# slimgroup/SetIntersectionProjection.jl

Measured on AMD Instinct MI355X. Metric: PARSDMM iterations/sec, higher is better.
Workload: dtype f32

## Files before the change

include/sipx.h:

```cpp
#ifndef SIPX_H
#define SIPX_H

#include <stdint.h>

#ifdef __cplusplus
extern "C" {
#endif

typedef struct sipx_ctx sipx_ctx;

enum { SIPX_F32 = 0, SIPX_F64 = 1 };

enum { SIPX_OP_IDENTITY = 0, SIPX_OP_DX = 1, SIPX_OP_DY = 2, SIPX_OP_DZ = 3, SIPX_OP_TV = 4,
       SIPX_OP_CSC = 5 ,
       SIPX_OP_TV_XY = 6  };

enum {
  SIPX_PROJ_BOUNDS      = 0,
  SIPX_PROJ_BOUNDS_VEC  = 1,
  SIPX_PROJ_L1          = 2,
  SIPX_PROJ_L2          = 3,
  SIPX_PROJ_ANNULUS     = 4,
  SIPX_PROJ_CARDINALITY = 5,
  SIPX_PROJ_PROX_L1     = 6,
// ... 60 lines not shown

const char* sipx_last_error(void);

int sipx_create(sipx_ctx** out, int dtype, int ndim, const int64_t* n, const double* h, int device);
void sipx_destroy(sipx_ctx* ctx);

int sipx_add_set(sipx_ctx* ctx, const sipx_set_desc* desc, const void* ata_R, const int64_t* ata_off, int d_i);

int sipx_set_rows(sipx_ctx* ctx, int set, int64_t* rows);
int sipx_num_terms(sipx_ctx* ctx, int* p, int* pp);

int sipx_finalize(sipx_ctx* ctx, const void* m, const double* rho_ini, int n_rho, double gamma_ini,
                  int feasibility_only, int zero_ini_guess, const void* x0, const void* const* l0,
                  const void* const* y0, double* feasibility_initial);

int sipx_reset(sipx_ctx* ctx, const void* m, const double* rho_ini, int n_rho, double gamma_ini, int zero_ini_guess,
               const void* x0, const void* const* l0, const void* const* y0, double* feasibility_initial);

int sipx_rhs_compose(sipx_ctx* ctx, const double* rho);
int sipx_argmin_x(sipx_ctx* ctx, int it, double* tol_ref_io, int64_t* cg_it, double* cg_relres, int* cg_flag);
enum { SIPX_YL_FEAS = 1,
       SIPX_YL_BB = 2,
       SIPX_YL_FIRST = 4   };
int sipx_update_y_l(sipx_ctx* ctx, int it, int flags, const double* rho, const double* gamma,
                    double* r_pri, double* r_dual, double* feas );
int sipx_log_scalars(sipx_ctx* ctx, double* obj, double* evol_x);
int sipx_adapt_rho_gamma(sipx_ctx* ctx, int adjust_rho, int adjust_gamma, double* rho_io, double* gamma_io);
int sipx_q_update(sipx_ctx* ctx, const double* rho_new, const double* rho_old);
int sipx_download(sipx_ctx* ctx, void* x, void* const* l, void* const* y);

int sipx_set_caller_stream(sipx_ctx* ctx, void* stream);
int sipx_finalize_dev(sipx_ctx* ctx, const void* m, const double* rho_ini, int n_rho, double gamma_ini, int feasibility_only,
                      int zero_ini_guess, const void* x0, const void* const* l0, const void* const* y0,
                      double* feasibility_initial);
int sipx_reset_dev(sipx_ctx* ctx, const void* m, const double* rho_ini, int n_rho, double gamma_ini, int zero_ini_guess,
                   const void* x0, const void* const* l0, const void* const* y0, double* feasibility_initial);
int sipx_download_dev(sipx_ctx* ctx, void* x, void* const* l, void* const* y);

int sipx_set_data(sipx_ctx* ctx, int set, const void* lb, const void* ub);
int sipx_set_data_dev(sipx_ctx* ctx, int set, const void* lb, const void* ub);
int sipx_io_bytes(sipx_ctx* ctx, int64_t* host_to_device, int64_t* device_to_host, int reset);

int sipx_warm_start_from(sipx_ctx* fine, sipx_ctx* coarse);

int sipx_parsdmm(sipx_ctx* ctx, const sipx_options* opt, sipx_log* log);
int sipx_parsdmm_begin(sipx_ctx* ctx, const sipx_options* opt, sipx_log* log);
int sipx_parsdmm_steps(sipx_ctx* ctx, int nsteps, int* done);

int sipx_cds_spmv(int dtype, int64_t N, int d, const void* R, const int64_t* off, const void* x, void* y, int device);
int sipx_apply_op(sipx_ctx* ctx, int op, const void* x, void* s);
int sipx_apply_op_adj(sipx_ctx* ctx, int op, const void* v, void* t);
int sipx_project(sipx_ctx* ctx, const sipx_set_desc* desc, void* v, int64_t len);
int sipx_segment_norms(sipx_ctx* ctx, int op, int mode, int dir, int norm, const void* x, void* out, int64_t* nseg);
int sipx_segment_norms_dev(sipx_ctx* ctx, int op, int mode, int dir, int norm, const void* x, void* out, int64_t* nseg);
int sipx_l21_norm(sipx_ctx* ctx, const void* x, void* out);
int sipx_l21_norm_dev(sipx_ctx* ctx, const void* x, void* out);
int sipx_l21_norms(sipx_ctx* ctx, int op, int mode, int dir, const void* x, void* out, int64_t* nseg);
int sipx_l21_norms_dev(sipx_ctx* ctx, int op, int mode, int dir, const void* x, void* out, int64_t* nseg);
int sipx_l21_joint_norm(sipx_ctx* ctx, const void* x, void* out);
int sipx_l21_joint_norm_dev(sipx_ctx* ctx, const void* x, void* out);
int sipx_l21_weighted_norm(sipx_ctx* ctx, int op, int joint, const void* x, const void* w, void* out);
int sipx_l21_weighted_norm_dev(sipx_ctx* ctx, int op, int joint, const void* x, const void* w, void* out);
int sipx_resample_nn(int dtype, int ndim, const int64_t* nc, const int64_t* nf, const void* in, void* out, int device);
int sipx_dwt(int dtype, int ndim, const int64_t* n, int inverse, const void* in, void* out, int device);

typedef struct {
  void* nuclear_norm; void* nuclear_Dx; void* nuclear_Dz; void* rank_095; void* TV; void* wavelet_l1; void* Dx_l1;
  void* Dz_l1; void* DFT_l1; void* DFT_card_095; void* TV_card_095; void* annulus; void* TV_annulus; void* D_l2;
  void* D_x_min; void* D_x_max; void* D_z_min; void* D_z_max; void* DCT_x_LB; void* DCT_x_UB; void* DCT_y_LB;
  void* DCT_y_UB; void* hist_min; void* hist_max; void* hist_TV_min; void* hist_TV_max;
} sipx_observations;
int sipx_learn_observations(int dtype, const int64_t* n, const double* h, int64_t n_train, const void* m_train,
                            const int64_t* strides, int64_t max_batch, sipx_observations* out, int device);
int sipx_get_Q(sipx_ctx* ctx, void* Q, int64_t* offsets, int* d);
int sipx_q_terms(sipx_ctx* ctx, int* bands, int* matrix_free);
int sipx_time_spmv(sipx_ctx* ctx, int reps, double* avg_ms);
int sipx_kernel_stats(sipx_ctx* ctx, int enable, int64_t* launches, double* total_ms);
const char* sipx_kernel_stats_json(sipx_ctx* ctx, int enable);
int sipx_debug_proj(sipx_ctx* ctx, int set, int which, double* out16);
void* sipx_stream(sipx_ctx* ctx);
void* sipx_dev_rhs(sipx_ctx* ctx);
void* sipx_dev_x(sipx_ctx* ctx);
int sipx_get_rhs(sipx_ctx* ctx, void* rhs);
int sipx_prox_l2s(int dtype, int64_t n, void* x, double rho, const void* m, int device);
int sipx_set_owned(sipx_ctx* ctx, const int32_t* owned);

int sipx_rccl_unique_id(void* id128);
#define SIPX_DECOMP_SETS 0
#define SIPX_DECOMP_SLAB 1
#define SIPX_DECOMP_SLAB_FULL 2
int sipx_set_decomp(sipx_ctx* ctx, int mode);
int sipx_set_comm_rccl(sipx_ctx* ctx, const void* id128, int world, int rank);
typedef struct {
  void* user;
  int32_t world, rank;
  int (*allreduce_sum)(void* user, void* buf, int64_t count, int32_t dtype, void* stream);
  int (*reduce_scatter_sum)(void* user, void* buf, int64_t chunk, int32_t dtype, void* stream);
  int (*allgather)(void* user, void* buf, int64_t chunk, int32_t dtype, void* stream);
  int (*halo_exchange)(void* user, const void* send_prev, void* recv_prev, int32_t prev, const void* send_next, void* recv_next,
                       int32_t next, int64_t count, int32_t dtype, void* stream);
  int (*scatter)(void* user, void* buf, int64_t chunk, int32_t dtype, int32_t root, void* stream);
  int (*gather)(void* user, void* buf, int64_t chunk, int32_t dtype, int32_t root, void* stream);
} sipx_comm;
int sipx_set_comm(sipx_ctx* ctx, const sipx_comm* comm);
int sipx_comm_info(sipx_ctx* ctx, int* nranks, int* rank, char* version, int version_len, int* decomposition);
int sipx_device_bytes(sipx_ctx* ctx, int64_t* context_bytes, int64_t* device_used, int64_t* device_total);
int sipx_slab(sipx_ctx* ctx, int64_t* row0, int64_t* row1, int64_t* chunk);

enum { SIPX_Q_CDS = 0, SIPX_Q_STENCIL = 1 };
int sipx_set_q_mode(sipx_ctx* ctx, int mode);
int sipx_apply_Q(sipx_ctx* ctx, const void* x, void* y);

#ifdef __cplusplus
}
#endif
#endif
```

setintersectionprojection.jl_amd/csrc/api.cpp:

```cpp
#include <string>

#include "comm.h"
#include "engine.h"
#include "learn.h"

struct sipx_ctx {
  sipx::EngineBase* e;
};

static thread_local std::string g_err;

#define SIPX_TRY(body)                   \
  try {                                  \
    body;                                \
    return 0;                            \
  } catch (const std::exception& ex) {   \
    g_err = ex.what();                   \
    return 1;                            \
  } catch (...) {                        \
    g_err = "unknown error";             \
    return 1;                            \
  }

extern "C" {
// ... 75 lines not shown
  SIPX_TRY({
    if (!fine || !coarse) throw std::runtime_error("null context");
    fine->e->warm_start_from(coarse->e);
  })
}
int sipx_parsdmm(sipx_ctx* c, const sipx_options* opt, sipx_log* log) { SIPX_TRY(c->e->parsdmm(opt, log)) }
int sipx_parsdmm_begin(sipx_ctx* c, const sipx_options* opt, sipx_log* log) { SIPX_TRY(c->e->parsdmm_begin(opt, log)) }
int sipx_parsdmm_steps(sipx_ctx* c, int nsteps, int* done) {
  SIPX_TRY({
    bool d = false;
    for (int k = 0; k < nsteps && !d; ++k) d = c->e->parsdmm_step();
    if (done) *done = d ? 1 : 0;
  })
}

int sipx_cds_spmv(int dtype, int64_t N, int d, const void* R, const int64_t* off, const void* x, void* y, int device) {
  SIPX_TRY(sipx::refresh_env_knobs(); sipx::cds_spmv_host(dtype, N, d, R, off, x, y, device))
}
int sipx_resample_nn(int dtype, int ndim, const int64_t* nc, const int64_t* nf, const void* in, void* out, int device) {
  SIPX_TRY(sipx::refresh_env_knobs(); sipx::resample_nn_host(dtype, ndim, nc, nf, in, out, device))
}
int sipx_dwt(int dtype, int ndim, const int64_t* n, int inverse, const void* in, void* out, int device) {
  SIPX_TRY(sipx::refresh_env_knobs(); sipx::dwt_host(dtype, ndim, n, inverse, in, out, device))
}
int sipx_learn_observations(int dtype, const int64_t* n, const double* h, int64_t n_train, const void* m_train,
                            const int64_t* strides, int64_t max_batch, sipx_observations* out, int device) {
  SIPX_TRY(sipx::refresh_env_knobs(); sipx::learn_observations_host(dtype, n, h, n_train, m_train, strides, max_batch, out, device))
}
int sipx_apply_op(sipx_ctx* c, int op, const void* x, void* s) { SIPX_TRY(c->e->apply_op(op, x, s, false)) }
int sipx_apply_op_adj(sipx_ctx* c, int op, const void* v, void* t) { SIPX_TRY(c->e->apply_op(op, v, t, true)) }
int sipx_project(sipx_ctx* c, const sipx_set_desc* d, void* v, int64_t len) { SIPX_TRY(sipx::refresh_env_knobs(); c->e->project(d, v, len)) }
int sipx_segment_norms(sipx_ctx* c, int op, int mode, int dir, int norm, const void* x, void* out, int64_t* nseg) {
  SIPX_TRY(sipx::refresh_env_knobs(); c->e->segment_norms(op, mode, dir, norm, x, out, nseg, false))
}
int sipx_segment_norms_dev(sipx_ctx* c, int op, int mode, int dir, int norm, const void* x, void* out, int64_t* nseg) {
  SIPX_TRY(sipx::refresh_env_knobs(); c->e->segment_norms(op, mode, dir, norm, x, out, nseg, true))
}
int sipx_l21_norm(sipx_ctx* c, const void* x, void* out) {
  SIPX_TRY(sipx::refresh_env_knobs(); c->e->l21_norms(SIPX_PROJ_L21, SIPX_OP_TV, SIPX_MODE_WHOLE, 0, x, out, nullptr, false, false))
}
int sipx_l21_norm_dev(sipx_ctx* c, const void* x, void* out) {
  SIPX_TRY(sipx::refresh_env_knobs(); c->e->l21_norms(SIPX_PROJ_L21, SIPX_OP_TV, SIPX_MODE_WHOLE, 0, x, out, nullptr, true, false))
}
int sipx_l21_norms(sipx_ctx* c, int op, int mode, int dir, const void* x, void* out, int64_t* nseg) {
  SIPX_TRY(sipx::refresh_env_knobs(); c->e->l21_norms(SIPX_PROJ_L21, op, mode, dir, x, out, nseg, false, true))
}
int sipx_l21_norms_dev(sipx_ctx* c, int op, int mode, int dir, const void* x, void* out, int64_t* nseg) {
  SIPX_TRY(sipx::refresh_env_knobs(); c->e->l21_norms(SIPX_PROJ_L21, op, mode, dir, x, out, nseg, true, true))
}
int sipx_l21_joint_norm(sipx_ctx* c, const void* x, void* out) {
  SIPX_TRY(sipx::refresh_env_knobs(); c->e->l21_norms(SIPX_PROJ_L21_JOINT, SIPX_OP_TV_XY, SIPX_MODE_WHOLE, 0, x, out, nullptr, false, false))
}
int sipx_l21_joint_norm_dev(sipx_ctx* c, const void* x, void* out) {
  SIPX_TRY(sipx::refresh_env_knobs(); c->e->l21_norms(SIPX_PROJ_L21_JOINT, SIPX_OP_TV_XY, SIPX_MODE_WHOLE, 0, x, out, nullptr, true, false))
}
int sipx_l21_weighted_norm(sipx_ctx* c, int op, int joint, const void* x, const void* w, void* out) {
  SIPX_TRY(sipx::refresh_env_knobs(); c->e->l21_weighted_norm(op, joint != 0, x, w, out, false))
}
int sipx_l21_weighted_norm_dev(sipx_ctx* c, int op, int joint, const void* x, const void* w, void* out) {
  SIPX_TRY(sipx::refresh_env_knobs(); c->e->l21_weighted_norm(op, joint != 0, x, w, out, true))
}
int sipx_get_Q(sipx_ctx* c, void* Q, int64_t* offsets, int* d) { SIPX_TRY(c->e->get_Q(Q, offsets, d)) }
int sipx_q_terms(sipx_ctx* c, int* bands, int* matrix_free) { SIPX_TRY(c->e->q_terms(bands, matrix_free)) }
int sipx_time_spmv(sipx_ctx* c, int reps, double* avg_ms) { SIPX_TRY(*avg_ms = c->e->time_spmv(reps)) }
int sipx_kernel_stats(sipx_ctx* c, int enable, int64_t* launches, double* total_ms) {
  SIPX_TRY(c->e->kernel_stats(enable, launches, total_ms))
}
const char* sipx_kernel_stats_json(sipx_ctx* c, int enable) {
  try {
    return c->e->kernel_stats_json(enable);
  } catch (const std::exception& ex) {
    g_err = ex.what();
    return nullptr;
  } catch (...) {
    g_err = "unknown error";
    return nullptr;
  }
}
int sipx_debug_proj(sipx_ctx* c, int set, int which, double* out16) { SIPX_TRY(c->e->debug_proj(set, which, out16)) }
void* sipx_stream(sipx_ctx* c) { return c->e->stream(); }
void* sipx_dev_rhs(sipx_ctx* c) { return c->e->dev_rhs(); }
void* sipx_dev_x(sipx_ctx* c) { return c->e->dev_x(); }
int sipx_get_rhs(sipx_ctx* c, void* rhs) { SIPX_TRY(c->e->get_rhs(rhs)) }
int sipx_prox_l2s(int dtype, int64_t n, void* x, double rho, const void* m, int device) {
  SIPX_TRY(sipx::refresh_env_knobs(); sipx::prox_l2s_host(dtype, n, x, rho, m, device))
}
int sipx_set_owned(sipx_ctx* c, const int32_t* owned) { SIPX_TRY(c->e->set_owned(owned)) }
int sipx_rccl_unique_id(void* id128) { SIPX_TRY(sipx::rccl_unique_id(id128)) }
int sipx_set_comm_rccl(sipx_ctx* c, const void* id128, int world, int rank) {
  SIPX_TRY({
    sipx::refresh_env_knobs();
    c->e->bind_device();
    c->e->set_comm(sipx::make_rccl_comm(id128, world, rank));
  })
}
int sipx_set_comm(sipx_ctx* c, const sipx_comm* comm) {
  SIPX_TRY({
    if (!comm) throw std::runtime_error("null communicator");
    sipx::refresh_env_knobs();
    c->e->set_comm(sipx::make_callback_comm(comm));
  })
}
int sipx_comm_info(sipx_ctx* c, int* nranks, int* rank, char* version, int version_len, int* decomposition) {
  SIPX_TRY(c->e->comm_info(nranks, rank, version, version_len, decomposition))
}
int sipx_device_bytes(sipx_ctx* c, int64_t* context_bytes, int64_t* device_used, int64_t* device_total) {
  SIPX_TRY(c->e->device_bytes(context_bytes, device_used, device_total))
}
int sipx_slab(sipx_ctx* c, int64_t* row0, int64_t* row1, int64_t* chunk) { SIPX_TRY(c->e->slab(row0, row1, chunk)) }
int sipx_set_q_mode(sipx_ctx* c, int mode) { SIPX_TRY(c->e->set_q_mode(mode)) }
int sipx_set_decomp(sipx_ctx* c, int mode) { SIPX_TRY(c->e->set_decomp(mode)) }
int sipx_apply_Q(sipx_ctx* c, const void* x, void* y) { SIPX_TRY(c->e->apply_Q(x, y)) }

}
```

setintersectionprojection.jl_amd/csrc/engine.cpp:

```cpp
#include "engine.h"
#include "comm.h"
#include "device_memory.h"
#include "dist_dft.h"
#include "ext_proj.h"
#include "host_prefault.h"
#include "set_config.h"
#include "solve_rules.h"
#include "sparse_granules.h"

#include <algorithm>
#include <array>
#include <chrono>
#include <cmath>
#include <cstdio>
#include <cstdlib>
#include <cstring>
#include <limits>
#include <thread>
#include <exception>

namespace sipx {

const LaunchObserver*& launch_observer() {
  static thread_local const LaunchObserver* obs = nullptr;
// ... 745 lines not shown
        s.cbuf = mem_.alloc<T>(s.Mpad, Mem::State);
      }
    }
    if (s.prox == SIPX_PROJ_BOUNDS_VEC) {
      s.lb = mem_.alloc<T>(s.Mpad); s.ub = mem_.alloc<T>(s.Mpad);
      if (!s.pend_lb) upload_rows(s, s.host_lb.data(), s.lb);
      if (!s.pend_ub) upload_rows(s, s.host_ub.data(), s.ub);
      if (s.pend_lb || s.pend_ub) {
        IoArgs<T> A;
        if (s.pend_lb) io_add_bounds(A, s, s.pend_lb, s.lb);
        if (s.pend_ub) io_add_bounds(A, s, s.pend_ub, s.ub);
        io_rows<T>(stream_, A, false, NB);
      }
    }
    if (!dev_io_ && l0 && l0[i]) upload_rows_ranged(s, (const T*)l0[i], s.l);
    if (!dev_io_ && y0 && y0[i]) upload_rows_ranged(s, (const T*)y0[i], s.y);
  }

  void create_lane(const FinalizePlan& P) {
    const bool one_rank = !comm_ && !mk_ && sweep_partial_;
    const bool slabbed = comm_ && slab_ && slab_loose_ && !mk_ && sweep_partial_;
    lane_set_ = -1;
    if (env_knobs().rank_lane && (one_rank || slabbed))
      for (int i = 0; i < p_n_ && lane_set_ < 0; ++i) {
        const SetState<T>& s = sets_[i];
        if (s.owned && !s.in_sweep && (one_rank ? !s.dist_ext : s.slab_ext) && s.ident && !s.custom && s.ext && s.rank_like()) lane_set_ = i;
      }
    if (lane_set_ < 0) return;
    int pr_least = 0, pr_greatest = 0;
    SIPX_HIP(hipDeviceGetStreamPriorityRange(&pr_least, &pr_greatest));
    SIPX_HIP(hipStreamCreateWithPriority(&lane_st_, hipStreamNonBlocking, pr_greatest));
    SIPX_HIP(hipEventCreateWithFlags(&lane_fork_, hipEventDisableTiming));
    SIPX_HIP(hipEventCreateWithFlags(&lane_ev_, hipEventDisableTiming));
    if (slab_) lane_v_ = (slab_local_ && !loose_whole_) ? loose_alloc(P.Npad) : mem_.alloc<T>((size_t)std::max<long long>(P.fullpad, sets_[lane_set_].Mpad), Mem::State);
    else lane_v_ = mem_.alloc<T>((size_t)sets_[lane_set_].Mpad, Mem::State);
  }

  void reset(const void* m, const double* rho_ini, int n_rho, double gamma_ini, int zero_ini_guess, const void* x0,
             const void* const* l0, const void* const* y0, double* feasibility_initial) override {
    need_final();
    if (comm_) throw std::runtime_error("sipx_reset is not available for a rank of a sharded solve (build a new context)");
    SIPX_HIP(hipSetDevice(device_));
    if (lane_thr_.joinable()) lane_thr_.join();
    lane_err_ = nullptr;
    SIPX_HIP(hipStreamSynchronize(stream_));
    for (hipStream_t q : pool_) if (q && q != stream_) SIPX_HIP(hipStreamSynchronize(q));
    if (lane_st_) SIPX_HIP(hipStreamSynchronize(lane_st_));
    if (cstream_) SIPX_HIP(hipStreamSynchronize(cstream_));
    const long long N = G_.N;
    mem_.zero_state(stream_);
    if (!dev_io_) {
      SIPX_HIP(hipMemcpyAsync(m_, m, N * sizeof(T), hipMemcpyHostToDevice, stream_));
      io_h2d_ += N * (long long)sizeof(T);
    }
    x_cur_ = 0; x_snap_ = -1;
    x_ = xr_[0]; xold_ = x_;
    init_rho_gamma(rho_ini, n_rho, gamma_ini);
    const bool warm = !zero_ini_guess;
    for (int i = 0; i < p_n_; ++i) {
      SetState<T>& s = sets_[i];
      s.snap = -1;
      s.searches_done = 0;
      std::fill(s.sums, s.sums + SLOTS, 0.0);
      s.bb_valid = false;
      s.last_rho = T(-1); s.last_gamma = T(-1);
      if (s.ps) K<T>::ps_init(stream_, s.ps, scr_i_);
      if (s.psf) K<T>::ps_init(stream_, s.psf, scr_i_);
      if (s.ext) { s.ext->set_stream(stream_); s.ext->reset(); }
      if (warm && !dev_io_ && l0 && l0[i]) upload_rows_ranged(s, (const T*)l0[i], s.l);
      if (warm && !dev_io_ && y0 && y0[i]) upload_rows_ranged(s, (const T*)y0[i], s.y);
    }
    if (dev_io_) {
      import_dev(m, warm ? x0 : nullptr, warm ? l0 : nullptr, warm ? y0 : nullptr);
    } else if (warm && x0) {
      SIPX_HIP(hipMemcpyAsync(x_, x0, Nx_ * sizeof(T), hipMemcpyHostToDevice, stream_));
      io_h2d_ += Nx_ * (long long)sizeof(T);
    }
    for (const PinnedBlock& b : pinned_blocks()) std::memset(*b.p, b.fill, b.bytes);
    sums_seq_ = 0; cg_seq_ = 0; spec_seq_ = 0;
    spec_searches_ = spec_fallbacks_ = spec_rounds_ = 0;
    batch_searches_ = batch_fallbacks_ = 0;
    for (long long& c : routes_) c = 0;
    head_done_ = false; rs_pending_ = false; sums_pending_ = false; merged_nslots_ = 0;
    rhs_fused_ = false; have_log_sums_ = false;
    obj_ss_ = evo_ss_ = xx_ss_ = 0;
    sums_flags_ = 0;
    marks_.reset();
    run_ = Run();
    assemble_Q();
    build_q_table();
    initial_feasibility(feasibility_initial);
  }

  void initial_feasibility(double* feasibility_initial) {
    feas_init_.assign(pp_n_, 0.0);
    for (int i = 0; i < pp_n_; ++i) {
      SetState<T>& s = sets_[i];
      if (s.dist_ext || s.slab_ext || s.slab_dft) {
        dist_feasibility(s, m_, fe2_part(i), i);
        continue;
      }
      if (s.fan) {
        SetArgs<T> a = set_args(s, rho_[i], gamma_[i], 0);
        a.x = m_;
        fan_feasibility(s, a, fe2_part(i));
        continue;
      }
      if (!s.owned) continue;
      if (slab_local_ && !s.two_pass && !s.ext_kind && !s.custom) {
        SetArgs<T> a = set_args(s, rho_[i], gamma_[i], 0);
        a.x = m_;
        K<T>::proj_dist_set(stream_, Gr_, a, 1, (const ProjScalars<T>*)nullptr, fe2_part(i));
        continue;
      }
      if (slab_ && !s.two_pass && comm_->rank != 0) continue;
      double* dst = fe2_part(i);
      const T* mm = s.comp == 2 ? w_ : m_;
      if (s.ext_kind) {
        SetArgs<T> a = set_args(s, rho_[i], gamma_[i], 0);
        a.x = mm;
        ext_feasibility(s, a, dst);
      } else if (s.custom) {
        custom_fwd(stream_, s, mm, s.sbuf);
        if (s.two_pass) {
          SetArgs<T> a = set_args(s, rho_[i], gamma_[i], 0);
          a.x = s.sbuf;
          K<T>::proj_scalars_set(stream_, s.gm, a, 1, s.psf, part_tmp_, maxpart_, scr_c_, s.Mtrue);
          K<T>::proj_dist_set(stream_, s.gm, a, 1, s.psf, dst);
        } else {
          proj_dist_grid<T>(stream_, s.gm, 0, s.dir, s.Mpad, s.sbuf, s.prox, s.plo, s.phi, s.lb, s.ub, nullptr, dst);
        }
      } else if (s.two_pass) {
        SetArgs<T> a = set_args(s, rho_[i], gamma_[i], 0);
        a.x = mm;
        SampleCtl cf;
        cf.host_ovf = (int*)hovf_ + i;
        cf.compact_cap = scr_c_len_;
        K<T>::proj_scalars_set(stream_, Gr_, a, 1, s.psf, part_tmp_, maxpart_, scr_c_, s.Mtrue, cf, hooks());
        K<T>::proj_dist_set(stream_, Gr_, a, 1, s.psf, dst);
      } else {
        K<T>::fwd(stream_, G_, s.nblk, s.dir, s.ih, mm, scr_v_);
        proj_dist_grid<T>(stream_, G_, s.nblk, s.dir, s.Mpad, scr_v_, s.prox, s.plo, s.phi, s.lb, s.ub, nullptr, dst);
      }
    }
    reduce_set_sums(p_n_ * SLOTS, YlPlan::Route::ByEvent);
    SIPX_HIP(hipStreamSynchronize(stream_));
    for (int i = 0; i < p_n_ && slab_; ++i)
      if (hovf_[i]) {
        hovf_[i] = 0;
        throw std::runtime_error("initial feasibility of set " + std::to_string(i) + ": the magnitudes inside the final bracket of the " + std::string(sets_[i].prox == PX_CARD ? "cardinality" : "l1") +
                                 " search, gathered over all ranks, exceed the exchange segment of " +
                                 std::to_string(hooks_.gcap) + " values per rank (slab decomposition) -- use the set decomposition for this problem");
      }
    for (int i = 0; i < pp_n_; ++i) {
      if (!sets_[i].owned && !comm_) continue;
      feas_init_[i] = (double)feas_value(hres_[i * SLOTS + SL_FE2], hres_[i * SLOTS + SL_SS2]);
    }
    if (feasibility_initial)
      for (int i = 0; i < pp_n_; ++i) feasibility_initial[i] = feas_init_[i];
  }

  void rhs_compose(const double* rho) override {
    need_final();
    ObserverGuard og(observer());
    head_done_ = false;
    if (rs_pending_) {
      SIPX_HIP(hipStreamWaitEvent(stream_, ev_c_[1], 0));
      rs_pending_ = false;
    }
    if (mk_) {
      for (int half = 0; half < 2; ++half) {
        T* out = rhs_ + (long long)half * G_.N;
        RhsBatch b(stream_, G_, out, false);
        for (int pass = 0; pass < 2; ++pass) {
          for (int i = 0; i < p_n_; ++i)
            if (sets_[i].comp == (pass == 0 ? half + 1 : 3)) b.add(sets_[i], (T)rho[i]);
          b.finish();
        }
        if (b.launched == 0) SIPX_HIP(hipMemsetAsync(out, 0, G_.N * sizeof(T), stream_));
      }
      return;
    }
    RhsBatch b(stream_, Gr_, rhs_, false);
    for (int i = 0; i < p_n_; ++i)
      if (sets_[i].owned && !sets_[i].custom) b.add(sets_[i], (T)rho[i]);
    if (b.launched == 0) b.flush();
    else b.finish();
    for (int i = 0; i < p_n_; ++i) {
      const SetState<T>& s = sets_[i];
      if (s.owned && s.custom) custom_adj_rhs(stream_, s, (T)rho[i]);
    }
    if (comm_ && !slab_) {
      SIPX_HIP(hipEventRecord(ev_c_[0], stream_));
      SIPX_HIP(hipStreamWaitEvent(cstream_, ev_c_[0], 0));
      comm_->reduce_scatter_sum(rhs_, (size_t)chunk_, dtype_code(), cstream_);
      SIPX_HIP(hipEventRecord(ev_c_[1], cstream_));
      rs_pending_ = true;
    }
  }

  void argmin_x_head() {
    if (rs_pending_) {
      SIPX_HIP(hipStreamWaitEvent(stream_, ev_c_[1], 0));
      rs_pending_ = false;
    }
    const long long r0 = r0_, r1 = r1_;
    const int dt = dtype_code();
    if (stencil_q_) K<T>::sq_resid(stream_, G_, sq_, x_, rhs_, p_, (T*)nullptr, (T*)nullptr, part_cg_);
    else K<T>::resid(stream_, Nx_, r0, r1, Q_, cds_, x_, rhs_, p_, (T*)nullptr, (T*)nullptr, part_cg_);
    mf_terms(x_, p_,  T(-1),  2, nullptr, nullptr);
    if (comm_) {
      comm_->allreduce_with_halo(part_cg_, (size_t)(2 * NB + merged_nslots_), SIPX_F64, p_ + r0, p_ + r0 - plane_, prev_, p_ + r1 - plane_,
                                 p_ + r1, next_, (size_t)plane_, dt, stream_);
      if (merged_nslots_ > 0) K<T>::copy_f64(stream_, dres_, hres_, merged_nslots_);
      merged_nslots_ = 0;
    }
    head_done_ = true;
  }

  void argmin_x(int it, double* tol_ref_io, int64_t* cg_it, double* cg_relres, int* cg_flag) override {
    need_final();
    ObserverGuard og(observer());
    if (!head_done_) argmin_x_head();
    head_done_ = false;
    const long long r0 = r0_, r1 = r1_, nloc = r1 - r0;
    const int dt = dtype_code();
    const long long hlo = (comm_ && prev_ >= 0) ? plane_ : 0, hhi = (comm_ && next_ >= 0) ? plane_ : 0;
    const unsigned seq = ++cg_seq_;
    K<T>::cg_begin(stream_, part_cg_, cg_dev_, cg_host_, it, (T)*tol_ref_io, seq, (unsigned long long*)ticket_);
    int tgt = 0;
    while (tgt == x_cur_ || tgt == x_snap_) ++tgt;
    T* const xn = xr_[tgt];
    auto enqueue = [&](int k) {
      CgState<T>* mirror = cg_host_ + (k & 1);
      if (stencil_q_) K<T>::sq_spmv_dot(stream_, G_, sq_, p_, Ap_, part_cg_, cg_dev_);
      else K<T>::spmv_dot(stream_, Nx_, r0, r1, Q_, cds_, p_, Ap_, part_cg_, cg_dev_);
      mf_terms(p_, Ap_, T(1),  1, p_, &cg_dev_->done);
      if (comm_) comm_->allreduce_sum(part_cg_, NB, SIPX_F64, stream_);
      K<T>::cg_update_xr(stream_, nloc, (k == 1 ? x_ : xn) + r0, xn + r0, (k == 1 ? p_ : r_) + r0, r_ + r0, p_ + r0, Ap_ + r0, part_cg_, cg_dev_, mirror, k,
                         (unsigned long long*)ticket_, hlo, hhi);
      if (comm_)
        comm_->allreduce_with_halo(part_cg_ + NB, NB, SIPX_F64, r_ + r0, r_ + r0 - plane_, prev_, r_ + r1 - plane_, r_ + r1, next_,
                                   (size_t)plane_, dt, stream_);
      K<T>::cg_update_p(stream_, nloc, p_ + r0, r_ + r0, part_cg_, cg_dev_, mirror, (unsigned long long*)ticket_, hlo, hhi);
    };
    auto enqueue_fused = [&](int k) {
      CgState<T>* mirror = cg_host_ + (k & 1);
      T* pk = (k & 1) ? p_ : p2_;
      T* pn = (k & 1) ? p2_ : p_;
      if (k == 1) K<T>::spmv_dot(stream_, Nx_, r0, r1, Q_, cds_, p_, Ap_, part_cg_, cg_dev_);
      K<T>::cg_update_xr(stream_, nloc, k == 1 ? x_ : xn, xn, k == 1 ? p_ : r_, r_, pk, Ap_, part_cg_, cg_dev_, mirror, k, (unsigned long long*)ticket_);
      K<T>::spmv_fused(stream_, Nx_, Q_, cds_, r_, pk, pn, Ap_, part_cg_, cg_dev_, mirror, (unsigned long long*)ticket_);
    };
    const size_t stat0 = samples_.size();
    const bool ahead = it > 1;
    auto enq = [&](int k) { if (cg_fused_) enqueue_fused(k); else enqueue(k); };
    if (ahead) enq(1);
    bool done = wait_ticket(seq, 0, cg_host_);
    const bool done_at_begin = done;
    CgState<T> fin;
    if (done) {
      fin = cg_host_[0];
      drop_samples_from(stat0);
      if (fin.flag == -9) SIPX_HIP(hipMemsetAsync(xn + r0 - hlo, 0, (nloc + hlo + hhi) * sizeof(T), stream_));
    } else {
      const int maxIter = 1000;
      int iter = 1;
      if (!ahead) enq(1);
      for (;;) {
        done = wait_ticket(seq, iter, cg_host_ + (iter & 1));
        if (done || iter == maxIter) break;
        enq(++iter);
      }
      fin = cg_host_[iter & 1];
    }
    cg_host_[0] = fin;
    const bool wrote = fin.flag == -9 || (!done_at_begin && !(fin.flag == -2 && fin.iters <= 1));
    if (wrote) {
      xold_ = x_;
      x_cur_ = tgt;
      x_ = xn;
    } else {
      xold_ = x_;
    }
// ... 964 lines not shown
        if (!s.two_pass || !s.in_sweep || s.prox != PX_L1 || s.custom || s.ext_kind) continue;
        SetArgs<T> a = set_args(s, (T)rho[i], (T)gamma[i], flags);
        if (a.flags & F_NOSPEC) continue;
        const bool rescaled = s.rescaled(a.rho);
        if (rescaled || search_ctl(i, rescaled, true).enable) { ok = false; break; }
        if (lm.ns == LEAN_MAX) break;
        const SetScratch scr = scratch_of(s);
        LeanSet<T>& S = lm.s[lm.ns++];
        S.a = a; S.a.ps = s.ps; S.ps = s.ps;
        S.compact = scr.cbuf; S.partials = scr.ptmp; S.maxpart = scr.mpart;
        who.push_back(i);
      }
      bool own = true;
      for (int i : who) own &= sets_[i].ptmp != nullptr && sets_[i].mpart != nullptr && sets_[i].cbuf != nullptr;
      if (ok && own && lm.ns >= 2) {
        K<T>::lean_multi(stream_, Gr_, lm);
        for (int i : who) lean_done[i] = 1;
      }
    }
    if (set_streams_) SIPX_HIP(hipEventRecord(ev_fork_, stream_));
    for (int i = 0; i < p_n_; ++i) {
      SetState<T>& s = sets_[i];
      if (!s.two_pass || !s.in_sweep) continue;
      SetArgs<T> a = set_args(s, (T)rho[i], (T)gamma[i], flags);
      hipStream_t q = s.st ? s.st : stream_;
      const SetScratch scr = scratch_of(s);
      if (q != stream_) SIPX_HIP(hipStreamWaitEvent(q, ev_fork_, 0));
      const bool rescaled = s.rescaled(a.rho);
      if (rescaled) K<T>::ps_rescale(q, s.ps, s.rescale_factor(a.rho));
      SampleCtl ctl = search_ctl(i, rescaled, true);
      ctl.lean_done = lean_done[i];
      K<T>::proj_scalars_set(q, Gr_, a, 0, s.ps, scr.ptmp, scr.mpart, scr.cbuf, s.Mtrue, ctl, nullptr);
      s.last_rho = a.rho;
      s.last_gamma = a.gamma;
      if (feas && i < pp_n_) {
        SampleCtl cf;
        cf.runs = env_knobs().l1_sample_runs;
        cf.enable = env_knobs().l1_sample && a.prox == PX_L1;
        K<T>::proj_scalars_set(q, Gr_, a, 1, s.psf, scr.ptmp, scr.mpart, scr.cbuf, s.Mtrue, cf, nullptr);
        K<T>::proj_dist_set(q, Gr_, a, 1, s.psf, fe2_part(i));
      }
    }
    join_set_streams([this](int i) { return sets_[i].two_pass && sets_[i].in_sweep; });
  }

  void sweep_launch(int flags, const double* rho, const double* gamma, MultiArgs<T>& ma, bool fuse_rhs) {
    const bool first = (flags & SIPX_YL_FIRST) != 0, bb = (flags & SIPX_YL_BB) != 0 && !first;
    ma.nblk = 0;
    std::vector<int> target(p_n_, 0);
    bool behind = false;
    for (int i = 0; i < p_n_; ++i) {
      SetState<T>& s = sets_[i];
      if (!s.in_sweep) { behind = true; target[i] = -1; continue; }
      SetArgs<T> a = set_args(s, (T)rho[i], (T)gamma[i], flags);
      target[i] = (!first && !bb && s.snap == 1) ? 2 : 0;
      if (target[i] == 2 && !s.y2) throw std::runtime_error("internal: the third y / l pair of the sweep was not allocated at sipx_finalize");
      T* ty = target[i] == 2 ? s.y2 : s.y0;
      T* tl = target[i] == 2 ? s.l2 : s.l0;
      for (int qb = 0; qb < s.nblk_or1(); ++qb) {
        MultiBlk<T>& B = ma.b[ma.nblk++];
        const long long off = (long long)qb * G_.N;
        B.y = s.y + off; B.l = s.l + off;
        B.yo = ty + off; B.lo = tl + off;
        B.lh0 = s.lh0 + off; B.s0 = s.s0 + off;
        B.y0 = a.y0 + off; B.l0 = a.l0 + off;
        B.ps = s.ps;
        B.dir = s.nblk == 0 ? -1 : s.dir[qb];
        B.set = i;
        B.first = qb == 0;
        B.last = qb == s.nblk_or1() - 1;
        B.dist = s.is_dist ? 1 : 0;
        B.feas_el = (i < pp_n_ && (s.prox == PX_BOUNDS || s.prox == PX_PROX_L1)) ? 1 : 0;
        B.ih = s.nblk == 0 ? T(0) : s.ih[qb];
        B.rho = a.rho; B.rho1 = a.rho1; B.gamma = a.gamma;
        B.prox = s.prox; B.plo = s.plo; B.phi = s.phi;
        B.in_rhs = behind ? 0 : 1;
      }
    }
    ma.x = x_; ma.m = m_; ma.xold = xold_;
    ma.x0 = (x0_mode_ && x_snap_ >= 0) ? xr_[x_snap_] : (x0_mode_ ? x_ : nullptr);
    ma.x0w = nullptr;
    ma.rhs = fuse_rhs ? rhs_ : nullptr;
    ma.partials = part_sets_;
    if (!K<T>::yl_multi(stream_, G_, ma)) throw std::runtime_error("internal: the fused y/l sweep refused a block list it was prepared for");
    rhs_fused_ = ma.rhs != nullptr;
    if (x0_mode_ && (first || bb)) x_snap_ = x_cur_;
    for (int i = 0; i < p_n_; ++i) {
      SetState<T>& s = sets_[i];
      if (target[i] < 0) continue;
      if (target[i] == 2) {
        std::swap(s.y, s.y2); std::swap(s.l, s.l2);
      } else {
        std::swap(s.y, s.y0); std::swap(s.l, s.l0);
        if (first || bb) s.snap = 0;
        else if (s.snap == 0) s.snap = 1;
      }
    }
  }

  void collect_set_sums(YlPlan::Route route, const double* rho, double* r_pri, double* r_dual, double* feas) {
    if (!sums_pending_) throw std::runtime_error("no y/l update is pending");
    sums_pending_ = false;
    const int flags = sums_flags_;
    if (route == YlPlan::Route::ByWord) wait_word(sums_word_, sums_seq_);
    else SIPX_HIP(hipEventSynchronize(sums_event_));
    have_log_sums_ = false;
    if (slab_) {
      for (int i = 0; i < p_n_; ++i) {
        if (!hovf_[i]) continue;
        for (int k = 0; k <= p_n_; ++k) hovf_[k] = 0;
        ProjScalars<T> h;
        SIPX_HIP(hipStreamSynchronize(stream_));
        char dbg[512];
        int at = 0;
        for (const ProjScalars<T>* d : {sets_[i].ps, sets_[i].psf}) {
          if (!d) continue;
          SIPX_HIP(hipMemcpy(&h, d, sizeof(h), hipMemcpyDeviceToHost));
          if (!h.gather_overflow) continue;
          at += std::snprintf(dbg + at, sizeof dbg - at, " [%s: bracket (%.9g, %.9g], refinement rounds %d, ||v||_1 %.6g, radius %.6g, speculative range (%.9g, %.9g]]",
                              d == sets_[i].ps ? "y/l update" : "feasibility estimate", h.lo, h.hi, h.rounds_used, h.asum, (double)sets_[i].phi, h.spec_lo, h.spec_hi);
        }
        dbg[at] = 0;
        throw std::runtime_error(std::string(sets_[i].prox == PX_CARD ? "cardinality search" : "l1 threshold search") + " of set " + std::to_string(i) + ": the magnitudes inside the final bracket, gathered over all "
                                 "ranks, exceed the exchange segment of " + std::to_string(hooks_.gcap) + " values per rank "
                                 "(slab decomposition) after the refinement rounds of the search; the iterate of this step is not valid -- "
                                 "use the set decomposition for this problem" + std::string(dbg));
      }
    }
    const bool all = comm_ != nullptr;
    for (int i = 0; i < p_n_; ++i) {
      SetState<T>& s = sets_[i];
      if (r_pri) r_pri[i] = 0;
      if (r_dual) r_dual[i] = 0;
      if (!s.owned && !all) continue;
      const double* h = hres_ + (size_t)i * SLOTS;
      std::copy(h, h + SLOTS, s.sums);
      if (r_pri) r_pri[i] = (double)(T)std::sqrt(h[SL_RPRI]);
      if (r_dual) r_dual[i] = (double)((T)rho[i] * (T)std::sqrt((s.comp == 3 ? 2.0 : 1.0) * (s.ident ? h[SL_DY] : h[SL_ADJ])));
      s.bb_valid = (flags & (SIPX_YL_BB | SIPX_YL_FIRST)) != 0;
      if (s.is_dist) {
        obj_ss_ = h[SL_OBJ]; evo_ss_ = h[SL_EVO]; xx_ss_ = h[SL_XX];
        if (mk_) { evo_ss_ = hres_[(size_t)p_n_ * SLOTS + SL_EVO]; xx_ss_ = hres_[(size_t)p_n_ * SLOTS + SL_XX]; }
        have_log_sums_ = true;
      }
    }
    if (all && !slab_dist_logs_) {
      const double* g = hres_ + (size_t)p_n_ * SLOTS;
      obj_ss_ = g[SL_OBJ]; evo_ss_ = g[SL_EVO]; xx_ss_ = g[SL_XX];
      have_log_sums_ = true;
    }
    if ((flags & SIPX_YL_FEAS) && feas) {
      for (int i = 0; i < pp_n_; ++i) {
        feas[i] = 0;
        if (!sets_[i].owned && !all) continue;
        const double* h = hres_ + (size_t)i * SLOTS;
        feas[i] = (sets_[i].two_pass || sets_[i].ext_kind) ? (double)feas_value(h[SL_FE2], h[SL_SS2])
                                                            : (double)feas_value(h[SL_FE], h[SL_SS]);
      }
    }
  }

  void log_scalars(double* obj, double* evol_x) override {
    need_final();
    ObserverGuard og(observer());
    if (!have_log_sums_) {
      K<T>::log3(stream_, G_.N, mk_ ? w_ : x_, m_, xold_, part_sets_);
      if (mk_) K<T>::log3(stream_, Nx_, x_, (const T*)nullptr, xold_, part_sets_ + (size_t)SLOTS * NB);
      K<T>::fin_sum(stream_, part_sets_, (mk_ ? 2 : 1) * SLOTS, nullptr, hres_);
// ... 430 lines not shown
      const long long c0 = slab_local_ ? std::max<long long>(0, wlo_) : 0, c1 = slab_local_ ? std::min<long long>(G_.N, whi_) : G_.N;
      if (c1 > c0) SIPX_HIP(hipMemcpyAsync(x_ + c0, m_ + c0, (c1 - c0) * sizeof(T), hipMemcpyDeviceToDevice, stream_));
    }
    if (mk_) SIPX_HIP(hipMemsetAsync(x_ + G_.N, 0, G_.N * sizeof(T), stream_));
    SIPX_HIP(hipStreamSynchronize(stream_));
    log->n_iter = 1;
    log->n_feas_rows = 1;
    log->stopped_feasible = 1;
    run_.done = true;
  }

  bool parsdmm_step() override {
    Run& R = run_;
    if (!R.active) throw std::runtime_error("sipx_parsdmm_steps: call sipx_parsdmm_begin first");
    if (R.done) return true;
    ObserverGuard og(observer());
    const int i = ++R.i;
    begin_step(i);
    x_step(i);
    const YlPlan plan = yl_step(i);
    queue_ahead(i, plan);
    collect_set_sums(plan.route, R.rho.data(), R.rpri.data(), R.rdual.data(), R.feas.data());
    record_log_row(i);
    if (stop_rule(i)) {
      finish_solve(i);
      return true;
    }
    next_rho(i);
    apply_rho(i);
    if (i == R.maxit) finish_solve(i);
    return R.done;
  }

  void begin_step(int i) {
    marks_.resolve(run_.log, i & 1);
    marks_.begin_step(i);
  }

  void x_step(int i) {
    Run& R = run_;
    if (!head_done_) marks_.open(i);
    if (!R.rhs_ready) {
      rhs_compose(R.rho.data());
      marks_.mark(1);
    }
    R.rhs_ready = false;
    int64_t cg_it; double relres; int flag;
    argmin_x(i, &R.tol_ref, &cg_it, &relres, &flag);
    R.log->cg_it[i - 1] = cg_it;
    R.log->cg_relres[i - 1] = relres;
    marks_.mark(2);
  }

  YlPlan yl_step(int i) {
    Run& R = run_;
    YlPlan plan;
    plan.collect_now = false;
    plan.fuse_rhs = i < R.maxit && !rho_may_change<T>(R.sw, i, pp_n_, R.rho.data(), p_n_);
    if (comm_) plan.route = plan.fuse_rhs ? YlPlan::Route::WithNextHead : YlPlan::Route::ByEvent;
    else plan.route = marks_.stride > 1 ? YlPlan::Route::ByWord : YlPlan::Route::ByEvent;
    yl_update(i, yl_flags(R.sw, i), R.rho.data(), R.gamma.data(), plan);
    marks_.mark(3);
    if (plan.route != YlPlan::Route::ByWord) sums_event_here();
    return plan;
  }
  void sums_event_here() {
    sums_event_ = marks_.last_event();
    if (sums_event_) return;
    SIPX_HIP(hipEventRecord(ev_sums_, stream_));
    sums_event_ = ev_sums_;
  }

  void queue_ahead(int i, const YlPlan& plan) {
    Run& R = run_;
    if (rhs_fused_) {
      R.rhs_ready = true;
    } else if (plan.fuse_rhs) {
      rhs_compose(R.rho.data());
      marks_.mark(1);
      R.rhs_ready = true;
    }
    if (!R.rhs_ready) return;
    marks_.open(i + 1);
    argmin_x_head();
    if (comm_) {
      marks_.mark(-1);
      sums_event_here();
    }
  }

  void record_log_row(int i) {
    Run& R = run_;
    sipx_log* log = R.log;
    const int p = p_n_, pp = pp_n_;
    HostSection t(log->timing_ms[3]);
    for (int k = 0; k < p; ++k) {
      log->r_pri[(size_t)(i - 1) * p + k] = R.rpri[k];
      log->r_dual[(size_t)(i - 1) * p + k] = R.rdual[k];
      log->rho[(size_t)(i - 1) * p + k] = R.rho[k];
      log->gamma[(size_t)(i - 1) * p + k] = R.gamma[k];
    }
    log->r_dual_total[i - 1] = seq_sum<T>(R.rdual.data(), p);
    log->r_pri_total[i - 1] = seq_sum<T>(R.rpri.data(), p);
    if (feas_due(i)) {
      for (int k = 0; k < pp; ++k) log->set_feasibility[(size_t)(R.counter - 1) * pp + k] = R.feas[k];
      R.counter += 1;
    }
    log_scalars(&log->obj[i - 1], &log->evol_x[i - 1]);
  }

  bool stop_rule(int i) {
    Run& R = run_;
    HostSection t(R.log->timing_ms[4]);
    const LogView view{R.log->set_feasibility, R.log->obj, R.log->evol_x, R.log->r_pri_total};
    return sipx::stop_rule<T>(view, i, R.counter, pp_n_, R.tol, R.sw);
  }

  void next_rho(int i) {
    Run& R = run_;
    HostSection t(R.log->timing_ms[5]);
    R.rho_new = R.rho;
    if (bb_due(R.sw, i)) adapt_rho_gamma(R.sw.adjust_rho, R.sw.adjust_gamma, R.rho_new.data(), R.gamma.data());
    const double* latest = R.log->set_feasibility + (size_t)(R.counter - 2) * pp_n_;
    sipx::next_rho<T>(R.sw, i, pp_n_, latest, R.rho_new.data(), p_n_);
  }

  void apply_rho(int i) {
    Run& R = run_;
    if (R.rhs_ready && R.rho_new != R.rho) throw std::runtime_error("internal: rho changed under a right-hand side queued ahead");
    bool changed = false;
    for (int k = 0; k < p_n_; ++k) changed |= R.rho_new[k] != R.rho[k];
    const bool rhs_due = i < R.maxit && !R.rhs_ready;
    if (rhs_due || changed) marks_.mark(-1);
    if (rhs_due) {
      rhs_compose(R.rho_new.data());
      marks_.mark(1);
      R.rhs_ready = true;
    }
    if (changed) {
      q_update(R.rho_new.data(), R.rho.data());
      marks_.mark(6);
    }
    R.rho = R.rho_new;
  }

  void finish_solve(int n_iter) {
    Run& R = run_;
    if (rs_pending_) {
      SIPX_HIP(hipStreamWaitEvent(stream_, ev_c_[1], 0));
      rs_pending_ = false;
    }
    marks_.resolve(R.log, 0);
    marks_.resolve(R.log, 1);
    R.log->n_iter = n_iter;
    R.log->n_feas_rows = R.counter;
    for (int k = 0; k < p_n_; ++k) { rho_[k] = (T)R.rho[k]; gamma_[k] = (T)R.gamma[k]; }
    R.rhs_ready = false;
    R.done = true;
    head_done_ = false;
  }

  void parsdmm(const sipx_options* opt, sipx_log* log) override {
    parsdmm_begin(opt, log);
    while (!parsdmm_step()) {
    }
  }
// ... 305 lines not shown
                    "\"bytes_moved\": %.0f, \"gated\": %s, \"inclusive\": %s}",
                    first ? "" : ", ", kernel_name(k), (long long)agg[k].launches, (long long)agg[k].noops, agg[k].ms, agg[k].bytes_survey,
                    agg[k].bytes_moved,
                    gated ? "true" : "false", k == KID_EXT ? "true" : "false");
      o += buf;
      first = false;
    }
    o += "], \"slab_searches\": {\"speculative_exchange\": " + std::to_string(spec_searches_) + ", \"fallbacks\": " +
         std::to_string(spec_fallbacks_) + ", \"refinement_rounds\": " + std::to_string(spec_rounds_) + "}";
    o += std::string(", \"sparse_arrays\": ") + (slab_local_ ? "true" : "false");
    {
      std::string loc, fan;
      for (int i = 0; i < p_n_; ++i) {
        if (sets_[i].slab_ext || sets_[i].slab_card || sets_[i].slab_dft) loc += (loc.empty() ? "" : ", ") + std::to_string(i);
        if (sets_[i].fan) fan += (fan.empty() ? "" : ", ") + std::to_string(i);
      }
      if (counting_)
        o += ", \"collectives\": {\"allreduce\": " + std::to_string(counting_->n_allreduce) + ", \"allreduce_with_halo\": " + std::to_string(counting_->n_grouped) +
             ", \"allgather\": " + std::to_string(counting_->n_allgather) + ", \"reduce_scatter\": " + std::to_string(counting_->n_reduce_scatter) +
             ", \"halo\": " + std::to_string(counting_->n_halo) + ", \"scatter_gather\": " + std::to_string(counting_->n_fan) +
             ", \"alltoall\": " + std::to_string(counting_->n_alltoall) + "}";
      o += ", \"slab_loose\": {\"slab_local_sets\": [" + loc + "], \"gathered_sets\": [" + fan + "], \"fan_exchanges\": " + std::to_string(fan_exchanges_) + "}";
    }
    {
      std::string t = selftest_;
      for (auto& ch : t) if (ch == '"' || ch == '\\' || (unsigned char)ch < 32) ch = ' ';
      o += ", \"comm_selftest\": \"" + t + "\"";
    }
    o += ", \"lane_set\": " + std::to_string(lane_set_);
    o += std::string(", \"q_table\": {\"on\": ") + (cds_.qtab ? "true" : "false") + ", \"reason\": \"" + qtab_reason_ + "\"}";
    o += ", \"batched_searches\": {\"searches\": " + std::to_string(batch_searches_) + ", \"fallbacks\": " + std::to_string(batch_fallbacks_) + "}";
    o += ", \"routes\": {";
    for (int r = 0; r < RT_COUNT; ++r) o += std::string(r ? ", \"" : "\"") + route_name(r) + "\": " + std::to_string(routes_[r]);
    o += "}";
    long long rc[4] = {project_rc_[0], project_rc_[1], project_rc_[2], project_rc_[3]};
    for (const auto& st : sets_) {
      if (!st.ext || st.ext_kind != EXT_RANK) continue;
      long long c[4];
      st.ext->route_counts(c);
      for (int q = 0; q < 4; ++q) rc[q] += c[q];
    }
    o += ", \"rank_route\": {\"calls\": " + std::to_string(rc[0]) + ", \"warm_started_subspace\": " + std::to_string(rc[1]) +
         ", \"full_decomposition\": " + std::to_string(rc[2]) + ", \"products_with_gram\": " + std::to_string(rc[3]) + "}";
    long long fc[4] = {0, 0, 0, 0};
    for (const auto& st : sets_) {
      if (!st.ext || st.ext_kind != EXT_L21_SEG) continue;
      long long c[4];
      st.ext->route_counts(c);
      fc[0] += c[0]; fc[1] = std::max(fc[1], c[1]); fc[3] += c[3];
    }
    o += ", \"l21_frames\": {\"passes_total\": " + std::to_string(fc[0]) + ", \"passes_max\": " + std::to_string(fc[1]) +
         ", \"frames\": " + std::to_string(fc[3]) + "}";
    long long wc[4] = {0, 0, 0, 0};
    for (const auto& st : sets_) {
      if (!st.ext || !st.weighted) continue;
      long long c[4];
      st.ext->route_counts(c);
      for (int q = 0; q < 4; ++q) wc[q] += c[q];
    }
    o += ", \"l21_weighted\": {\"passes\": " + std::to_string(wc[0]) + ", \"flag_reads\": " + std::to_string(wc[1]) +
         ", \"calls\": " + std::to_string(wc[2]) + ", \"groups\": " + std::to_string(wc[3]) + "}}";
    if (!peek) start_stats(enable);
    return o.c_str();
  }
  double stat_pair_overhead_ms() const { return stat_pair_ms_; }

  void debug_proj(int set, int which, double* o) override {
    need_final();
    for (int k = 0; k < 16; ++k) o[k] = 0;
    if (set < 0 || set >= p_n_) throw std::runtime_error("set index out of range");
    const ProjScalars<T>* d = (which & 1) ? sets_[set].psf : sets_[set].ps;
    if (!d) return;
    ProjScalars<T> h;
    SIPX_HIP(hipStreamSynchronize(stream_));
    SIPX_HIP(hipMemcpy(&h, d, sizeof(h), hipMemcpyDeviceToHost));
    o[0] = h.need; o[1] = h.theta; o[2] = h.theta_prev; o[3] = h.hw; o[4] = h.spec_lo; o[5] = h.spec_hi; o[6] = h.lo;
    o[7] = h.hi; o[8] = h.asum; o[9] = h.vmax; o[10] = h.dbg[0]; o[11] = h.dbg[1]; o[12] = h.dbg[2]; o[13] = h.dbg[3];
    o[14] = h.refine;
    o[15] = h.lean + 2 * h.dbg_sampled;
    if (which & 2) { o[4] = h.samp_theta; o[5] = h.samp_lo; o[6] = h.samp_hi; o[7] = h.samp_c; }
  }

  void* stream() override { return (void*)stream_; }
  void* dev_rhs() override { return rhs_; }
  void* dev_x() override { return x_; }
  void get_rhs(void* out) override {
    need_final();
    if (slab_local_ && comm_->world > 1) throw std::runtime_error("a slab-decomposed context holds its planes of rhs only");
    SIPX_HIP(hipStreamSynchronize(stream_));
    SIPX_HIP(hipMemcpy(out, rhs_, Nx_ * sizeof(T), hipMemcpyDeviceToHost));
  }

 private:
  struct KSample { int kid; double bytes_survey, bytes_moved; };
  struct KAgg { long long launches = 0, noops = 0; double ms = 0, bytes_survey = 0, bytes_moved = 0; };
  hipEvent_t stat_event(size_t i) {
    while (stat_ev_.size() <= i) {
      hipEvent_t e;
      SIPX_HIP(hipEventCreate(&e));
      stat_ev_.push_back(e);
    }
    return stat_ev_[i];
  }
  static void obs_begin(void* user, int kid, hipStream_t s, double bytes_survey, double bytes_moved) {
    auto* e = static_cast<Engine<T>*>(user);
    if (e->stats_mode_ == 0 || (e->stats_mode_ == 1 && kid != KID_CDS_DOT && kid != KID_SQ_DOT)) return;
    const size_t i = e->samples_.size();
    e->samples_.push_back(KSample{kid, bytes_survey, bytes_moved});
    e->open_.push_back(i);
    SIPX_HIP(hipEventRecord(e->stat_event(2 * i), s));
  }
  static void obs_end(void* user, int kid, hipStream_t s) {
    auto* e = static_cast<Engine<T>*>(user);
    if (e->stats_mode_ == 0 || (e->stats_mode_ == 1 && kid != KID_CDS_DOT && kid != KID_SQ_DOT)) return;
    if (e->open_.empty()) return;
    const size_t i = e->open_.back();
    e->open_.pop_back();
    if (i < e->samples_.size()) SIPX_HIP(hipEventRecord(e->stat_event(2 * i + 1), s));
  }
  static void obs_route(void* user, int route) {
    if (route >= 0 && route < RT_COUNT) static_cast<Engine<T>*>(user)->routes_[route] += 1;
  }
  void drop_samples_from(size_t n) {
    if (n < samples_.size()) samples_.resize(n);
    open_.clear();
  }
  void sync_all_streams() {
    SIPX_HIP(hipStreamSynchronize(stream_));
    for (hipStream_t q : pool_) if (q != stream_) SIPX_HIP(hipStreamSynchronize(q));
    if (cstream_) SIPX_HIP(hipStreamSynchronize(cstream_));
  }
  static bool gated_kernel(int k) {
    return k == KID_PASS_FIRST || k == KID_PASS_LEAN || k == KID_PASS_PROBE || k == KID_PASS_COMPACT || k == KID_SAMPLE ||
           k == KID_DECIDE || k == KID_CDS_FUSED || k == KID_CG_XR || k == KID_CG_P || k == KID_SLOT_SUMS;
  }
  std::vector<KAgg> aggregate_samples() {
    sync_all_streams();
    std::vector<KAgg> agg(KID_COUNT);
    for (size_t i = 0; i < samples_.size(); ++i) {
      float ms = 0;
      if (hipEventElapsedTime(&ms, stat_ev_[2 * i], stat_ev_[2 * i + 1]) != hipSuccess) { (void)hipGetLastError(); continue; }
      KAgg& a = agg[samples_[i].kid];
      const double t = (double)ms - stat_pair_ms_;
      a.launches += 1;
      a.ms += t > 0 ? t : 0;
      const bool noop = gated_kernel(samples_[i].kid) && samples_[i].bytes_moved > 0 && t * 1e-3 < samples_[i].bytes_moved / 16e12;
      a.noops += noop ? 1 : 0;
      a.bytes_survey += noop ? 0.0 : samples_[i].bytes_survey;
      a.bytes_moved += noop ? 0.0 : samples_[i].bytes_moved;
    }
    return agg;
  }
  void start_stats(int mode) {
    samples_.clear();
    open_.clear();
    stats_mode_ = 0;
    if (mode) {
      std::vector<float> gap;
      for (int k = 0; k < 16; ++k) {
        SIPX_HIP(hipEventRecord(stat_event(2 * k), stream_));
        SIPX_HIP(hipEventRecord(stat_event(2 * k + 1), stream_));
      }
      SIPX_HIP(hipStreamSynchronize(stream_));
      for (int k = 0; k < 16; ++k) {
        float ms = 0;
        SIPX_HIP(hipEventElapsedTime(&ms, stat_ev_[2 * k], stat_ev_[2 * k + 1]));
        gap.push_back(ms);
      }
      std::sort(gap.begin(), gap.end());
      stat_pair_ms_ = gap[gap.size() / 2];
    }
    stats_mode_ = mode;
  }
// ... 502 lines not shown
    explicit DevIoGuard(bool* flag) : f(flag) { *f = true; }
    ~DevIoGuard() { *f = false; }
  };
  Grid G_;
  T ih_[3];
  std::vector<SetState<T>> sets_;
  std::vector<int32_t> owned_;
  bool finalized_ = false, feasibility_only_ = false, any_ncvx_ = false;
  int p_n_ = 0, pp_n_ = 0;
  std::vector<T> rho_, gamma_;
  std::vector<double> feas_init_;
  T *p_base_ = nullptr, *m_base_ = nullptr, *r_base_ = nullptr, *p2_base_ = nullptr, *p2_ = nullptr;
  bool cg_fused_ = false;
  int n_mfree_ = 0;
  long long halo_ = 0;
  T *x_ = nullptr, *xold_ = nullptr, *rhs_ = nullptr, *m_ = nullptr, *r_ = nullptr, *p_ = nullptr, *Ap_ = nullptr;
  T *Q_ = nullptr, *scr_v_ = nullptr, *scr_c_ = nullptr, *maxpart_ = nullptr;
  long long* scr_i_ = nullptr;
  long long scr_c_len_ = 0;
  T* scr_w_ = nullptr;
  T *loose_v_ = nullptr, *loose_w_ = nullptr;
  bool loose_whole_ = false;
  bool need_idx_ = false, need_ext_ = false;
  CdsArgs cds_;
  bool set_streams_ = true;
  hipEvent_t ev_fork_ = nullptr, ev_fork2_ = nullptr;
  std::vector<hipStream_t> pool_;
  bool search_streams_ = false;
  int search_next_ = 0;
  int n_set_streams_ = 2, pool_next_ = 0;
  bool mk_ = false;
  long long Nx_ = 0;
  T *w_base_ = nullptr, *w_ = nullptr;
  StencilQ<T> sq_{};
  bool stencil_q_ = false;
  double *part_cg_ = nullptr, *part_tmp_ = nullptr, *part_sets_ = nullptr;
  CgState<T>*cg_dev_ = nullptr, *cg_host_ = nullptr;
  double* hres_ = nullptr;
  volatile unsigned long long* sums_word_ = nullptr;
  unsigned* sums_ticket_ = nullptr;
  unsigned long long sums_seq_ = 0;
  volatile int* hlean_ = nullptr;
  volatile int* hovf_ = nullptr;
  volatile unsigned* hverd_ = nullptr;
  unsigned spec_seq_ = 0;
  long long spec_searches_ = 0, spec_fallbacks_ = 0, spec_rounds_ = 0;
  int lane_set_ = -1;
  hipStream_t lane_st_ = nullptr;
  hipEvent_t lane_fork_ = nullptr, lane_ev_ = nullptr;
  T* lane_v_ = nullptr;
  std::thread lane_thr_;
  std::exception_ptr lane_err_;
  long long lane_sample_ = -1;
  SetArgs<T> lane_args_;
  bool sweep_partial_ = false, has_loose_ = false;
  bool sweep_plain_ = false;
  bool search_batch_ = false;
  long long batch_searches_ = 0, batch_fallbacks_ = 0;
  long long routes_[RT_COUNT] = {};
  long long project_rc_[4] = {0, 0, 0, 0};
  T* fbuf_ = nullptr;
  bool yl_multi_ = true;
  bool x0_mode_ = false;
  T *xr_base_[3] = {nullptr, nullptr, nullptr}, *xr_[3] = {nullptr, nullptr, nullptr};
  int x_cur_ = 0, x_snap_ = -1;
  bool rhs_fused_ = false;
  hipEvent_t sums_event_ = nullptr;
  std::unique_ptr<Comm> comm_;
  CountingComm* counting_ = nullptr;
  long long plane_ = 0, chunk_ = 0, r0_ = 0, r1_ = 0, qr0_ = 0, qr1_ = 0;
  int prev_ = -1, next_ = -1;
  hipStream_t cstream_ = nullptr;
  hipEvent_t ev_c_[2] = {nullptr, nullptr};
  bool rs_pending_ = false;
  double* dres_ = nullptr;
  hipEvent_t ev_sums_ = nullptr, ev_cgb_ = nullptr;
  bool sums_pending_ = false;
  T* qtab_ = nullptr;
  bool q_stale_ = false;
  std::string qtab_reason_ = "not built";
  DeviceMemory mem_;
  bool slab_dist_logs_ = false;
  bool lean_multi_ = false;
  bool head_done_ = false;
  int merged_nslots_ = 0;
  int sums_flags_ = 0;
  volatile unsigned long long* ticket_ = nullptr;
  unsigned cg_seq_ = 0;
  bool slab_req_ = false, slab_ = false;
  hipStream_t fan_st_ = nullptr;
  hipEvent_t fan_fork_ = nullptr;
  double* fan_ptmp_ = nullptr;
  T *fan_mpart_ = nullptr, *fan_c_ = nullptr;
  long long fan_exchanges_ = 0;
  bool slab_loose_ = false;
  bool slab_full_req_ = false, slab_local_ = false;
  std::string selftest_ = "none", mapped_why_;
  double* agree_buf_ = nullptr;
  bool selftest_mapped_failed_ = false, selftest_alltoall_failed_ = false;
  std::string a2a_why_;
  long long wlo_ = 0, whi_ = 0;
  Grid Gr_, Gyl_;
  ChainHooks hooks_;
  T* gbuf_ = nullptr;
  double *stage_ = nullptr, *sstage_ = nullptr;
  const ChainHooks* hooks() const { return slab_ ? &hooks_ : nullptr; }
  double obj_ss_ = 0, evo_ss_ = 0, xx_ss_ = 0;
  bool have_log_sums_ = false;
  hipEvent_t cg_ev_[2] = {nullptr, nullptr};
  std::vector<hipEvent_t> stat_ev_;
  std::vector<KSample> samples_;
  std::vector<size_t> open_;
  int stats_mode_ = 0;
  LaunchObserver obs_{this, &Engine<T>::obs_begin, &Engine<T>::obs_end, &Engine<T>::obs_route};
  std::string stats_json_;
  double stat_pair_ms_ = 0;
};

EngineBase* make_engine(int dtype, int ndim, const int64_t* n, const double* h, int device) {
  const int count = hip_device_count();
  if (device < 0 || device >= count) throw std::runtime_error("libsipx: device index out of range");
  if (dtype == SIPX_F32) return new Engine<float>(ndim, n, h, device);
  if (dtype == SIPX_F64) return new Engine<double>(ndim, n, h, device);
  throw std::runtime_error("dtype must be SIPX_F32 or SIPX_F64");
}

template <typename T>
static void cds_spmv_T(int64_t N, int d, const void* R, const int64_t* off, const void* x, void* y) {
  if (d < 1 || d > MAXD) throw std::runtime_error("cds_spmv: band count out of range");
  long long H = 4;
  for (int b = 0; b < d; ++b) H = std::max<long long>(H, std::llabs((long long)off[b]));
  H = (H + 3) / 4 * 4;
  DeviceMemory tmp;
  T* dR = tmp.alloc<T>((size_t)N * d, Mem::NoFill);
  T* dxb = tmp.alloc<T>(N + 2 * H);
  T* dx = dxb + H;
  T* dy = tmp.alloc<T>(N);
  SIPX_HIP(hipMemcpy(dR, R, (size_t)N * d * sizeof(T), hipMemcpyHostToDevice));
  SIPX_HIP(hipMemcpy(dx, x, N * sizeof(T), hipMemcpyHostToDevice));
  CdsArgs a;
  a.d = d;
  for (int b = 0; b < d; ++b) a.off[b] = off[b];
  Grid g;
  g.n[0] = N; g.n[1] = 1; g.n[2] = 1; g.N = N; g.st[0] = 1; g.st[1] = N; g.st[2] = N;
  K<T>::spmv(nullptr, g, N, dR, a, dx, dy);
  SIPX_HIP(hipDeviceSynchronize());
  SIPX_HIP(hipMemcpy(y, dy, N * sizeof(T), hipMemcpyDeviceToHost));
}

template <typename T>
static void resample_T(int ndim, const int64_t* nc, const int64_t* nf, const void* in, void* out) {
  long long c[3] = {1, 1, 1}, f[3] = {1, 1, 1};
  for (int q = 0; q < ndim && q < 3; ++q) { c[q] = nc[q]; f[q] = nf[q]; }
  const long long Nc = c[0] * c[1] * c[2], Nf = f[0] * f[1] * f[2];
  if (Nc < 1 || Nf < 1) throw std::runtime_error("resample: empty array");
  DeviceMemory tmp;
  T* di = tmp.alloc<T>(Nc, Mem::NoFill);
  T* dout = tmp.alloc<T>(Nf, Mem::NoFill);
  SIPX_HIP(hipMemcpy(di, in, Nc * sizeof(T), hipMemcpyHostToDevice));
  resample_nn<T>(nullptr, c, f, di, dout);
  SIPX_HIP(hipDeviceSynchronize());
  SIPX_HIP(hipMemcpy(out, dout, Nf * sizeof(T), hipMemcpyDeviceToHost));
}
void resample_nn_host(int dtype, int ndim, const int64_t* nc, const int64_t* nf, const void* in, void* out, int device) {
  hip_device_count();
  if (ndim < 1 || ndim > 3) throw std::runtime_error("resample: ndim must be 1..3");
// ... 61 lines not shown
```

setintersectionprojection.jl_amd/csrc/engine.h:

```cpp
#pragma once
#include <memory>
#include <stdexcept>
#include <string>
#include <vector>

#include "../../include/sipx.h"
#include "sipx_common.h"

namespace sipx {

struct Comm;

struct EngineBase {
  virtual ~EngineBase() {}
  virtual int add_set(const sipx_set_desc* d, const void* ata_R, const int64_t* ata_off, int d_i) = 0;
  virtual int64_t set_rows(int set) = 0;
  virtual void num_terms(int* p, int* pp) = 0;
  virtual void finalize(const void* m, const double* rho_ini, int n_rho, double gamma_ini, int feasibility_only,
                        int zero_ini_guess, const void* x0, const void* const* l0, const void* const* y0,
                        double* feasibility_initial) = 0;
  virtual void reset(const void* m, const double* rho_ini, int n_rho, double gamma_ini, int zero_ini_guess, const void* x0,
                     const void* const* l0, const void* const* y0, double* feasibility_initial) = 0;
  virtual void rhs_compose(const double* rho) = 0;
  virtual void argmin_x(int it, double* tol_ref_io, int64_t* cg_it, double* cg_relres, int* cg_flag) = 0;
  virtual void update_y_l(int it, int flags, const double* rho, const double* gamma, double* r_pri, double* r_dual,
                          double* feas) = 0;
  virtual void log_scalars(double* obj, double* evol_x) = 0;
  virtual void adapt_rho_gamma(int adjust_rho, int adjust_gamma, double* rho_io, double* gamma_io) = 0;
  virtual void q_update(const double* rho_new, const double* rho_old) = 0;
  virtual void download(void* x, void* const* l, void* const* y) = 0;
  virtual void warm_start_from(EngineBase* coarse) = 0;
  virtual void finalize_dev(const void* m, const double* rho_ini, int n_rho, double gamma_ini, int feasibility_only,
                            int zero_ini_guess, const void* x0, const void* const* l0, const void* const* y0,
                            double* feasibility_initial) = 0;
  virtual void reset_dev(const void* m, const double* rho_ini, int n_rho, double gamma_ini, int zero_ini_guess, const void* x0,
                         const void* const* l0, const void* const* y0, double* feasibility_initial) = 0;
  virtual void download_dev(void* x, void* const* l, void* const* y) = 0;
  virtual void set_caller_stream(void* stream) = 0;
  virtual void set_data(int set, const void* lb, const void* ub, bool on_device) = 0;
  virtual void io_bytes(int64_t* host_to_device, int64_t* device_to_host, int reset) = 0;
  virtual void parsdmm(const sipx_options* opt, sipx_log* log) = 0;
  virtual void parsdmm_begin(const sipx_options* opt, sipx_log* log) = 0;
  virtual bool parsdmm_step() = 0;
  virtual void apply_op(int op, const void* x, void* s, bool adjoint) = 0;
  virtual void project(const sipx_set_desc* d, void* v, int64_t len) = 0;
  virtual void segment_norms(int op, int mode, int dir, int norm, const void* x, void* out, int64_t* nseg, bool on_device) = 0;
  virtual void l21_norms(int proj, int op, int mode, int dir, const void* x, void* out, int64_t* nseg, bool on_device, bool query) = 0;
  virtual void l21_weighted_norm(int op, bool joint, const void* x, const void* w, void* out, bool on_device) = 0;
  virtual void get_Q(void* Q, int64_t* offsets, int* d) = 0;
  virtual void apply_Q(const void* x, void* y) = 0;
  virtual void q_terms(int* bands, int* matrix_free) = 0;
  virtual double time_spmv(int reps) = 0;
  virtual void kernel_stats(int enable, int64_t* launches, double* total_ms) = 0;
  virtual const char* kernel_stats_json(int enable) = 0;
  virtual void debug_proj(int set, int which, double* out16) = 0;
  virtual void* stream() = 0;
  virtual void* dev_rhs() = 0;
  virtual void* dev_x() = 0;
  virtual void get_rhs(void* out) = 0;
  virtual void set_owned(const int32_t* owned) = 0;
  virtual void set_q_mode(int mode) = 0;
  virtual void set_decomp(int mode) = 0;
  virtual void set_comm(Comm* c) = 0;
  virtual void comm_info(int* nranks, int* rank, char* version, int version_len, int* decomposition) = 0;
  virtual void bind_device() = 0;
  virtual void device_bytes(int64_t* context_bytes, int64_t* device_used, int64_t* device_total) = 0;
  virtual void slab(int64_t* row0, int64_t* row1, int64_t* chunk) = 0;
};

EngineBase* make_engine(int dtype, int ndim, const int64_t* n, const double* h, int device);
void resample_nn_host(int dtype, int ndim, const int64_t* nc, const int64_t* nf, const void* in, void* out, int device);
void dwt_host(int dtype, int ndim, const int64_t* n, int inverse, const void* in, void* out, int device);
void prox_l2s_host(int dtype, int64_t n, void* x, double rho, const void* m, int device);
void cds_spmv_host(int dtype, int64_t N, int d, const void* R, const int64_t* off, const void* x, void* y, int device);

}
```

setintersectionprojection.jl_amd/csrc/kernels_cds.hip:

```cpp
#include <cstdlib>
#include <stdexcept>
#include <string>

#include "sipx_device.h"
#define SIPX_CG_GRID launch_blocks(3)
#ifndef SIPX_F64_VEC
#define SIPX_F64_VEC 2
#endif

namespace sipx {

template <typename T, int V>
struct LoadStored {
  const T* __restrict__ x;
  __device__ __forceinline__ Vec<T, V> operator()(long long c) const { return ldv_u<T, V>(x + c); }
};
template <typename T, int V>
struct LoadFused {
  const T* __restrict__ r;
  const T* __restrict__ p;
  T beta;
  __device__ __forceinline__ Vec<T, V> operator()(long long c) const {
    const Vec<T, V> rv = ldv_u<T, V>(r + c), pv = ldv_u<T, V>(p + c);
    Vec<T, V> o;
// ... 16 lines not shown
      if (a.sym) {
        rv[b] = a.off[b] >= 0 ? ldv<T, V>(R + (long long)b * N + r)
                              : ldv_u<T, V>(R + (long long)a.partner[b] * N + r + a.off[b]);
      } else {
        rv[b] = ldv_nt<T, V>(R + (long long)b * N + r);
      }
      xv[b] = xl(r + a.off[b]);
    }
#pragma unroll
    for (int b = 0; b < D; ++b) {
      const long long c = r + a.off[b];
#pragma unroll
      for (int k = 0; k < V; ++k) {
        const T t = acc[k] + rv[b].v[k] * xv[b].v[k];
        acc[k] = (c + k >= 0 && c + k < N) ? t : acc[k];
      }
    }
  } else {
    for (int b = 0; b < d; ++b) {
      const long long c = r + a.off[b];
      const Vec<T, V> rv = !a.sym ? ldv_nt<T, V>(R + (long long)b * N + r)
                                  : (a.off[b] >= 0 ? ldv<T, V>(R + (long long)b * N + r)
                                                   : ldv_u<T, V>(R + (long long)a.partner[b] * N + c));
      const Vec<T, V> xv = xl(c);
#pragma unroll
      for (int k = 0; k < V; ++k) {
        const T t = acc[k] + rv.v[k] * xv.v[k];
        acc[k] = (c + k >= 0 && c + k < N) ? t : acc[k];
      }
    }
  }
}

template <typename T, int V, int D, int MODE>
__global__ __launch_bounds__(BLOCK) void k_cds(long long N, long long r0, long long r1, const T* __restrict__ R, CdsArgs a,
                                               const T* __restrict__ x, T* __restrict__ y, const T* __restrict__ b,
                                               T* __restrict__ pout, T* __restrict__ xold, double* __restrict__ partials,
                                               const int* __restrict__ done) {
  if (MODE == 1 && *done) return;
  const long long nvec = r1 / V;
  double acc0 = 0, acc1 = 0;
  for (long long vi = r0 / V + (long long)blockIdx.x * BLOCK + threadIdx.x; vi < nvec; vi += (long long)gridDim.x * BLOCK) {
    const long long r = vi * V;
    T s[V];
    cds_rows<T, V, D>(N, R, a, LoadStored<T, V>{x}, r, s);
    if (MODE == 0) {
      Vec<T, V> o;
#pragma unroll
      for (int k = 0; k < V; ++k) o.v[k] = s[k];
      stv_nt<T, V>(y + r, o);
    } else if (MODE == 1) {
      const Vec<T, V> pv = ldv<T, V>(x + r);
      Vec<T, V> o;
#pragma unroll
      for (int k = 0; k < V; ++k) {
        o.v[k] = s[k];
        acc0 += (double)pv.v[k] * (double)s[k];
      }
      stv_nt<T, V>(y + r, o);
    } else {
      const Vec<T, V> bv = ldv<T, V>(b + r);
      const Vec<T, V> xv = ldv<T, V>(x + r);
      Vec<T, V> o;
#pragma unroll
      for (int k = 0; k < V; ++k) {
        o.v[k] = bv.v[k] - s[k];
        acc0 += (double)o.v[k] * (double)o.v[k];
        acc1 += (double)bv.v[k] * (double)bv.v[k];
      }
      stv<T, V>(y + r, o);
      if (pout) stv<T, V>(pout + r, o);
      if (xold) stv<T, V>(xold + r, xv);
    }
  }
  if (MODE == 1) {
    double acc[1] = {acc0};
    block_reduce_store<1>(acc, partials, 0);
  } else if (MODE == 2) {
    double acc[2] = {acc0, acc1};
    block_reduce_store<2>(acc, partials, 0);
  }
}

constexpr int march_role(int ord, int b) {
  constexpr int o1[7] = {0, 1, 2, 3, 4, 5, 6}, o2[7] = {0, 5, 3, 1, 2, 4, 6};
  return ord == 1 ? o1[b] : o2[b];
}
template <typename T>
__device__ __forceinline__ T ata_value(const Grid& G, int nblk, const int* dir, const T* ihs, long long o, const Coord& c) {
  T val = (nblk == 0 && o == 0) ? T(1) : T(0);
  for (int q = 0; q < nblk; ++q) {
    const int d = dir[q];
    const T ih = ihs[q], nih = -ih;
    const int cc = coord_of(c, d);
    const long long st = G.st[d];
    if (o == 0) {
      if (cc > 0) val = val + ih * ih;
      if (cc < G.n[d] - 1) val = val + nih * nih;
    } else if (o == st) {
      if (cc < G.n[d] - 1) val = val + nih * ih;
    } else if (o == -st) {
      if (cc > 0) val = val + ih * nih;
    }
  }
  return val;
}

constexpr int QP_MAXB = 9, QP_MAXT = 8, QP_TAB = 160;
struct QPlanTerm {
  int kind;
  int nblk;
  int dir[3];
  int tab;
};
template <typename T>
struct QPlan {
  int nbands;
  int col[QP_MAXB], nterms[QP_MAXB];
  QPlanTerm t[QP_MAXB][QP_MAXT];
  int ntab;
  T tab[QP_TAB];
};

struct NoExtra {};
template <typename T>
struct QTab {
  const T* tab;
};
template <typename X>
struct IsQTab { static constexpr bool value = false; };
template <typename T>
struct IsQTab<QTab<T>> { static constexpr bool value = true; };
template <typename T>
__device__ __forceinline__ void load_class_tab(const QTab<T>& u, T* tab) {
  for (int i = threadIdx.x; i < QT_N; i += blockDim.x) tab[i] = u.tab[i];
}
template <typename X, typename T>
__device__ __forceinline__ void load_class_tab(const X&, T*) {}
__device__ __forceinline__ int line_class(long long c, long long n) { return c == 0 ? 0 : (c == n - 1 ? 2 : 1); }
template <typename T, int V>
__device__ __forceinline__ Vec<T, V> tab_row(const T* tab, int role, int cyz, long long i0, long long n1) {
  const T* e = tab + 27 * role + cyz;
  const T first = e[0], mid = e[1], last = e[2];
  Vec<T, V> v;
#pragma unroll
  for (int k = 0; k < V; ++k) v.v[k] = i0 + k == 0 ? first : (i0 + k == n1 - 1 ? last : mid);
  return v;
}
__device__ __forceinline__ void publish_ticket(unsigned long long* ticket, unsigned seq, int iter, int done);
constexpr int MARCH_NT = 512;
template <typename T, int V, int ORD, int MODE, typename X>
__global__ __launch_bounds__(MARCH_NT) void k_cds_march(long long n1, long long n2, long long n3, long long z0, long long z1, const T* __restrict__ R0,
                                                        const T* __restrict__ R1, const T* __restrict__ R2, const T* __restrict__ R3,
                                                        const T* __restrict__ x, T* __restrict__ y, const T* __restrict__ b,
                                                        T* __restrict__ pout, T* __restrict__ xold, double* __restrict__ partials,
                                                        const int* __restrict__ done, int lgLX, int tiles_x, int tiles_y, int zchunk,
                                                        long long items, CgState<T>* __restrict__ st, CgState<T>* __restrict__ host,
                                                        unsigned long long* ticket, X extra) {
  constexpr bool TAB = IsQTab<X>::value;
  if (MODE == 1 && *done) return;
  T beta = T(0);
  if (MODE == 3) {
    if (st->done) return;
    const double ss = block_sum_partials_n<MARCH_NT>(partials + NB);
    const T rr = (T)ss;
    const T res = (T)sqrt(ss) / st->nr0;
    const bool conv = res <= st->tol;
    beta = rr / st->gamma;
    if (blockIdx.x == 0 && threadIdx.x == 0) {
      st->ss = ss;
      st->res_last = res;
      if (conv) { st->flag = 0; st->done = 1; } else { st->beta = beta; }
      st->rr = rr;
      *host = *st;
      publish_ticket(ticket, st->seq, st->iters, conv ? 1 : 0);
    }
    if (conv) return;
  }
  auto ldx = [&](long long at) -> Vec<T, V> {
    Vec<T, V> v = ldv<T, V>(x + at);
    if (MODE == 3) {
      const Vec<T, V> pv = ldv<T, V>(b + at);
#pragma unroll
      for (int k = 0; k < V; ++k) v.v[k] = v.v[k] + beta * pv.v[k];
    }
    return v;
  };
  auto ldx1 = [&](long long at) -> T { return MODE == 3 ? x[at] + beta * b[at] : x[at]; };
  __shared__ T sx[2][V][MARCH_NT], sr[TAB ? 1 : 2][TAB ? 1 : V][TAB ? 1 : MARCH_NT];
  __shared__ T ctab[TAB ? QT_N : 1];
  if (TAB) {
    load_class_tab(extra, ctab);
    __syncthreads();
  }
  const int tid = threadIdx.x, LX = 1 << lgLX, tx = tid & (LX - 1), ty = tid >> lgLX, TY = MARCH_NT >> lgLX;
  const long long st1 = n1, st2 = n1 * n2, N = st2 * n3;
  const long long tiles = (long long)tiles_x * tiles_y;
  double acc0 = 0, acc1 = 0;
  for (long long item = blockIdx.x; item < items; item += gridDim.x) {
    const long long zc = item / tiles, tile = item - zc * tiles;
    const int tile_y = (int)(tile / tiles_x), tile_x = (int)(tile - (long long)tile_y * tiles_x);
    const long long i0 = ((long long)tile_x * LX + tx) * V, j = (long long)tile_y * TY + ty;
    const bool active = i0 < n1 && j < n2;
    const long long k0 = z0 + zc * zchunk, k1 = (k0 + zchunk < z1) ? k0 + zchunk : z1;
    const unsigned go = active ? (unsigned)(i0 + st1 * j) : 0u;
    __syncthreads();
    Vec<T, V> xm = zerov<T, V>(), x0 = zerov<T, V>(), rzm = zerov<T, V>();
    if (active) {
      xm = ldx(st2 * (k0 - 1) + go);
      x0 = ldx(st2 * k0 + go);
      if (k0 > 0 && TAB) {
        rzm = tab_row<T, V>(ctab, 3, 3 * line_class(j, n2) + 9 * line_class(k0 - 1, n3), i0, n1);
      } else if (k0 > 0) {
        rzm = ldv<T, V>(R3 + st2 * (k0 - 1) + go);
      }
    }
    for (long long kz = k0; kz < k1; ++kz) {
      const int par = (int)(kz & 1);
      const long long pz = st2 * kz;
      Vec<T, V> xp = zerov<T, V>(), r0 = xp, r1 = xp, r2 = xp, r3 = xp, bv = xp;
      const int cz = TAB ? line_class(kz, n3) : 0, cyz = TAB ? 3 * line_class(j, n2) + 9 * cz : 0;
      const int cyz_up = !TAB ? 0 : (j > 0 ? 3 * line_class(j - 1, n2) + 9 * cz : 3 * line_class(n2 - 1, n2) + 9 * line_class(kz - 1, n3));
      if (active) {
        xp = ldx(pz + st2 + go);
        if constexpr (TAB) {
          r0 = tab_row<T, V>(ctab, 0, cyz, i0, n1);
          r1 = tab_row<T, V>(ctab, 1, cyz, i0, n1);
          r2 = tab_row<T, V>(ctab, 2, cyz, i0, n1);
          r3 = tab_row<T, V>(ctab, 3, cyz, i0, n1);
        } else {
          r0 = ldv_nt<T, V>(R0 + pz + go);
// ... 991 lines not shown
```

setintersectionprojection.jl_amd/csrc/kernels_multi.hip:

```cpp
#include <cstdlib>
#include <stdexcept>
#include <string>
#include <type_traits>

#include "sipx_device.h"

namespace sipx {

#ifndef SIPX_MULTI_PREFETCH
#define SIPX_MULTI_PREFETCH 1
#endif
#ifndef SIPX_MULTI_VF
#define SIPX_MULTI_VF 4
#endif
#ifndef SIPX_MULTI_WAVES
#define SIPX_MULTI_WAVES 1
#endif
constexpr int MULTI_NT = 256;

enum { LK_I = 1, LK_X = 2, LK_Y = 3, LK_Z = 4, LK_D = 5 };
constexpr unsigned long long lay_blk(int kind, bool last) { return (unsigned long long)(kind | (last ? 8 : 0)); }
constexpr unsigned long long lay_pack(unsigned long long b0, unsigned long long b1 = 0, unsigned long long b2 = 0, unsigned long long b3 = 0,
                                      unsigned long long b4 = 0, unsigned long long b5 = 0, unsigned long long b6 = 0,
                                      unsigned long long b7 = 0) {
  return b0 | (b1 << 4) | (b2 << 8) | (b3 << 12) | (b4 << 16) | (b5 << 20) | (b6 << 24) | (b7 << 28);
}
constexpr int lay_kind(unsigned long long L, int b) { return (int)((L >> (4 * b)) & 7); }
constexpr bool lay_last(unsigned long long L, int b) { return ((L >> (4 * b)) & 8) != 0; }
constexpr bool lay_first(unsigned long long L, int b) { return b == 0 || lay_last(L, b - 1); }
constexpr int lay_count(unsigned long long L) {
  int n = 0;
  while (n < MULTI_MAXB && lay_kind(L, n) != 0) ++n;
  return n;
}
constexpr int lay_count_kind(unsigned long long L, int kind) {
  int n = 0;
  for (int b = 0; b < MULTI_MAXB; ++b) n += lay_kind(L, b) == kind;
  return n;
}
constexpr int lay_index_among(unsigned long long L, int b, int kind) {
  int n = 0;
  for (int c = 0; c < b; ++c) n += lay_kind(L, c) == kind;
  return n;
}
constexpr int lay_sets(unsigned long long L) {
  int n = 0;
  for (int b = 0; b < MULTI_MAXB; ++b) n += (lay_kind(L, b) != 0 && lay_last(L, b)) ? 1 : 0;
  return n;
}

template <typename T>
struct UniProx {
  T lo, hi, theta, scale;
  int fill;
};
template <typename T>
__device__ __forceinline__ UniProx<T> make_uniprox(const MultiBlk<T>& B) {
  UniProx<T> u;
  u.lo = -(T)INFINITY; u.hi = (T)INFINITY; u.theta = T(0); u.scale = T(1); u.fill = 0;
  if (B.prox == PX_BOUNDS) { u.lo = B.plo; u.hi = B.phi; }
  if (B.prox == PX_L1) u.theta = B.ps->theta;
  if (B.prox == PX_PROX_L1) u.theta = T(1) / B.phi;
  if (B.prox == PX_L2 || B.prox == PX_ANNULUS) { u.scale = B.ps->scale; u.fill = B.ps->fill; }
  return u;
}

template <typename T, int VV, int KIND>
__device__ __forceinline__ void multi_block_update(const MultiBlk<T>& B, const UniProx<T>& pc, const Vec<T, VV>& xc, const Vec<T, VV>& xn,
                                                   const bool (&valid)[VV], const Vec<T, VV>& yv, const Vec<T, VV>& lv, const Vec<T, VV>& mv,
                                                   Vec<T, VV>& yn, Vec<T, VV>& ln, T (&rp)[VV], T (&sv)[VV]) {
  const bool relax = !(B.gamma == T(1));
  const T gam = B.gamma, omg = T(1) - B.gamma, nih = -B.ih;
#pragma unroll
  for (int k = 0; k < VV; ++k) {
    T s;
    if constexpr (KIND == LK_I || KIND == LK_D) {
      s = xc.v[k];
    } else {
      const T d = nih * xc.v[k] + B.ih * xn.v[k];
      s = valid[k] ? d : T(0);
    }
    const T yo = yv.v[k], lo = lv.v[k];
    const T xh = relax ? (gam * s + omg * yo) : s;
    const T v = xh - lo * B.rho1;
    T y1;
    if constexpr (KIND == LK_D) {
      y1 = (T)((double)(v * B.rho + mv.v[k]) / ((double)B.rho + 1.0));
    } else {
      const T t = soft_thr(v, pc.theta);
      const T q = pc.fill ? pc.scale : t * pc.scale;
      const T c = q < pc.hi ? q : pc.hi;
      y1 = pc.lo > c ? pc.lo : c;
      if constexpr (KIND != LK_I) { if (!valid[k]) y1 = T(0); }
    }
    rp[k] = y1 - s;
    ln.v[k] = relax ? (lo + B.rho * (y1 - xh)) : (lo + B.rho * rp[k]);
    yn.v[k] = y1;
    sv[k] = s;
  }
}

template <int I, int N, typename F>
__device__ __forceinline__ void static_for(F&& f) {
  if constexpr (I < N) {
    f(std::integral_constant<int, I>{});
    static_for<I + 1, N>(f);
  }
}

template <typename T, int V, unsigned long long L, bool FULL, bool X0>
__global__ __launch_bounds__(MULTI_NT, SIPX_MULTI_WAVES) void k_yl_multi(Grid G, MultiArgs<T> a, int lgLX, int tiles_x, int tiles_y, int zchunk,
                                                       long long items, long long jlo, long long jhi, long long jsum, int xsplit) {
  constexpr int NBLK = lay_count(L), NY = lay_count_kind(L, LK_Y), NZ = lay_count_kind(L, LK_Z);
  constexpr int NSETS = lay_sets(L), NI = lay_count_kind(L, LK_I);
  constexpr int NACC = FULL ? 6 * NSETS : 1;
  __shared__ double lacc[NACC][MULTI_NT / 4];
  __shared__ T ybuf[2][NY > 0 ? NY : 1][2][V][MULTI_NT];
  const bool f_first = FULL && (a.flags & F_FIRST) != 0, f_bb = FULL && (a.flags & F_BB) != 0 && !f_first;
  const bool f_feas = FULL && (a.flags & F_FEAS) != 0;
  if constexpr (FULL) {
#pragma unroll
    for (int q = 0; q < NACC; ++q) lacc[q][threadIdx.x >> 2] = 0.0;
  }
  const int tid = threadIdx.x, LX = 1 << lgLX, tx = tid & (LX - 1), ty = tid >> lgLX, TY = MULTI_NT >> lgLX;
  const long long n1 = G.n[0], n2 = G.n[1], n3 = G.n[2], st1 = G.st[1], st2 = G.st[2];
  const bool fuse_rhs = a.rhs != nullptr;

  UniProx<T> pc[NBLK];
#pragma unroll
  for (int b = 0; b < NBLK; ++b) pc[b] = make_uniprox<T>(a.b[b]);
  double acc_rp[NBLK], acc_du[NBLK];
#pragma unroll
  for (int b = 0; b < NBLK; ++b) acc_rp[b] = acc_du[b] = 0;
  double acc_obj = 0, acc_evo = 0, acc_xx = 0;
  double acc_fe[NI > 0 ? NI : 1], acc_ss[NI > 0 ? NI : 1];
#pragma unroll
  for (int q = 0; q < (NI > 0 ? NI : 1); ++q) acc_fe[q] = acc_ss[q] = 0;

  const long long tiles = (long long)tiles_x * tiles_y;
  for (long long item = blockIdx.x; item < items; item += gridDim.x) {
    const long long zc = item / tiles, tile = item - zc * tiles;
    const int tile_y = (int)(tile / tiles_x), tile_x = (int)(tile - (long long)tile_y * tiles_x);
    const long long i0 = xsplit ? (((long long)tile_x * TY + ty) * LX + tx) * V : ((long long)tile_x * LX + tx) * V;
    const long long j = xsplit ? jlo + tile_y : jlo + (long long)tile_y * TY + ty;
    const bool active = i0 < n1 && j < jhi;
    const long long k0 = a.zlo + zc * zchunk, k1 = (k0 + zchunk < a.zhi) ? k0 + zchunk : a.zhi;
    const unsigned go = active ? (unsigned)(i0 + st1 * j) : 0u;
    bool vx[V], mxm[V];
#pragma unroll
    for (int k = 0; k < V; ++k) { vx[k] = (i0 + k) < n1 - 1; mxm[k] = (i0 + k) > 0; }
    const bool vy = j < n2 - 1, mym = j > 0;
    if constexpr (NY > 0) __syncthreads();

    T zw[NZ > 0 ? NZ : 1][V], zd[NZ > 0 ? NZ : 1][V];
    static_for<0, NBLK>([&](auto bc) {
      constexpr int b = decltype(bc)::value;
      if constexpr (lay_kind(L, b) == LK_Z) {
        constexpr int zi = lay_index_among(L, b, LK_Z);
        const MultiBlk<T>& B = a.b[b];
#pragma unroll
        for (int k = 0; k < V; ++k) zw[zi][k] = zd[zi][k] = T(0);
        if (active && k0 > 0) {
          const long long pz = st2 * (k0 - 1);
          const Vec<T, V> xc = ldv<T, V>(a.x + pz + go), xn = ldv_u<T, V>(a.x + pz + st2 + go);
          const Vec<T, V> yv = ldv<T, V>(B.y + pz + go), lv = ldv<T, V>(B.l + pz + go);
          bool valid[V];
#pragma unroll
          for (int k = 0; k < V; ++k) valid[k] = true;
          Vec<T, V> yn, ln;
          T rp[V], sv[V];
          multi_block_update<T, V, LK_Z>(B, pc[b], xc, xn, valid, yv, lv, zerov<T, V>(), yn, ln, rp, sv);
#pragma unroll
          for (int k = 0; k < V; ++k) { zw[zi][k] = B.rho * yn.v[k] + ln.v[k]; zd[zi][k] = yn.v[k] - yv.v[k]; }
        }
      }
    });

    Vec<T, V> xnext = active ? ldv<T, V>(a.x + st2 * k0 + go) : zerov<T, V>();
    constexpr bool x0mode = FULL && X0;
    Vec<T, V> x0next = (x0mode && f_bb && active) ? ldv<T, V>(a.x0 + st2 * k0 + go) : zerov<T, V>();
    for (long long kz = k0; kz < k1; ++kz) {
      const int par = (int)(kz & 1);
      const long long pz = st2 * kz;
      const Vec<T, V> xc = xnext;
      const bool vz = kz < n3 - 1, mzm = kz > 0;
      const bool own = kz >= a.zsum && j >= jsum;
      Vec<T, V> xpx = zerov<T, V>(), xpy = zerov<T, V>();
      Vec<T, V> yv[NBLK], lv[NBLK], mv = zerov<T, V>(), xo = zerov<T, V>();
#pragma unroll
      for (int b = 0; b < NBLK; ++b) { yv[b] = zerov<T, V>(); lv[b] = zerov<T, V>(); }
      if (active) {
        xnext = ldv_u<T, V>(a.x + pz + st2 + go);
        if constexpr (lay_count_kind(L, LK_X) > 0) xpx = ldv_u<T, V>(a.x + pz + 1 + go);
        if constexpr (NY > 0) xpy = ldv_u<T, V>(a.x + pz + st1 + go);
        if constexpr (SIPX_MULTI_PREFETCH && !FULL) {
#pragma unroll
          for (int b = 0; b < NBLK; ++b) {
            yv[b] = ldv_nt<T, V>(a.b[b].y + pz + go);
            lv[b] = ldv_nt<T, V>(a.b[b].l + pz + go);
          }
        }
        if constexpr (lay_count_kind(L, LK_D) > 0) { mv = ldv<T, V>(a.m + pz + go); xo = ldv<T, V>(a.xold + pz + go); }
      }
      Vec<T, V> x0c = x0next, x0px = zerov<T, V>(), x0py = zerov<T, V>();
      if constexpr (FULL) {
        if (x0mode && f_bb && active) {
          x0next = ldv_u<T, V>(a.x0 + pz + st2 + go);
          if constexpr (lay_count_kind(L, LK_X) > 0) x0px = ldv_u<T, V>(a.x0 + pz + 1 + go);
          if constexpr (NY > 0) x0py = ldv_u<T, V>(a.x0 + pz + st1 + go);
        }
        if (x0mode && a.x0w && (f_bb || f_first) && active) stv_nt<T, V>(a.x0w + pz + go, xc);
      }
      T wv[NBLK][V], dv[NBLK][V];
      static_for<0, NBLK>([&](auto bc) {
        constexpr int b = decltype(bc)::value;
        constexpr int KIND = lay_kind(L, b);
        const MultiBlk<T>& B = a.b[b];
#pragma unroll
        for (int k = 0; k < V; ++k) wv[b][k] = dv[b][k] = T(0);
        if (active) {
          if constexpr (!SIPX_MULTI_PREFETCH || FULL) {
            yv[b] = ldv_nt<T, V>(B.y + pz + go);
            lv[b] = ldv_nt<T, V>(B.l + pz + go);
          }
          bool valid[V];
#pragma unroll
          for (int k = 0; k < V; ++k) valid[k] = KIND == LK_X ? vx[k] : (KIND == LK_Y ? vy : (KIND == LK_Z ? vz : true));
          const Vec<T, V>& xn = KIND == LK_X ? xpx : (KIND == LK_Y ? xpy : xnext);
          Vec<T, V> yn, ln;
          T rp[V], sv[V];
          multi_block_update<T, V, KIND>(B, pc[b], xc, xn, valid, yv[b], lv[b], mv, yn, ln, rp, sv);
          if constexpr (FULL) {
            constexpr int si = lay_sets(L & ((1ull << (4 * b)) - 1ull));
            Vec<T, V> lh, svv;
#pragma unroll
            for (int k = 0; k < V; ++k) {
              lh.v[k] = lv[b].v[k] + B.rho * (yv[b].v[k] - sv[k]);
              svv.v[k] = sv[k];
            }
            if (f_bb) {
              const Vec<T, V> a0 = ldv_nt<T, V>(B.lh0 + pz + go), b0 = ldv_nt<T, V>(B.y0 + pz + go), d0 = ldv_nt<T, V>(B.l0 + pz + go);
              Vec<T, V> c0;
              if (x0mode) {
                const Vec<T, V>& x0n = KIND == LK_X ? x0px : (KIND == LK_Y ? x0py : x0next);
#pragma unroll
                for (int k = 0; k < V; ++k) {
                  if constexpr (KIND == LK_I || KIND == LK_D) {
                    c0.v[k] = x0c.v[k];
                  } else {
                    const T d = (-B.ih) * x0c.v[k] + B.ih * x0n.v[k];
                    c0.v[k] = valid[k] ? d : T(0);
                  }
                }
              } else {
                c0 = ldv_nt<T, V>(B.s0 + pz + go);
              }
              double q6[6] = {0, 0, 0, 0, 0, 0};
#pragma unroll
              for (int k = 0; k < V; ++k) {
                const T dlh = lh.v[k] - a0.v[k], dH = sv[k] - c0.v[k], dl = ln.v[k] - d0.v[k], dG = -(yn.v[k] - b0.v[k]);
                q6[0] += (double)dH * (double)dlh;
                q6[1] += (double)dH * (double)dH;
                q6[2] += (double)dlh * (double)dlh;
                q6[3] += (double)dl * (double)dl;
                q6[4] += (double)dG * (double)dG;
                q6[5] += (double)dG * (double)dl;
              }
#pragma unroll
              for (int q = 0; q < 6; ++q) {
                double v = own ? q6[q] : 0.0;
                v += dpp_hop<0xb1, 0xf>(v);
                v += dpp_hop<0x4e, 0xf>(v);
                if ((tid & 3) == 0) lacc[6 * si + q][tid >> 2] += v;
              }
            }
            if (f_bb || f_first) {
              stv_nt<T, V>(B.lh0 + pz + go, lh);
              if (!x0mode) stv_nt<T, V>(B.s0 + pz + go, svv);
            }
            if constexpr (KIND == LK_I) {
              if (f_feas && B.feas_el && own) {
                constexpr int ii = lay_index_among(L, b, LK_I);
                double fe = 0, ss = 0;
#pragma unroll
                for (int k = 0; k < V; ++k) {
                  const T t = soft_thr(sv[k], pc[b].theta);
                  const T q = pc[b].fill ? pc[b].scale : t * pc[b].scale;
                  const T c = q < pc[b].hi ? q : pc[b].hi;
                  const T psv = pc[b].lo > c ? pc[b].lo : c;
                  const T d = psv - sv[k];
                  fe += (double)d * (double)d;
                  ss += (double)sv[k] * (double)sv[k];
                }
                acc_fe[ii] += fe;
// ... 40 lines not shown
#pragma unroll
          for (int k = 0; k < V; ++k) tr[k] = td[k] = T(0);
        }
        if constexpr (KIND == LK_I || KIND == LK_D) {
#pragma unroll
          for (int k = 0; k < V; ++k) tr[k] = wv[b][k];
        } else {
          T pw[V], pd[V];
          bool mm[V], mc[V];
          if constexpr (KIND == LK_X) {
            T lw = __shfl_up(wv[b][V - 1], 1, 64), ld = __shfl_up(dv[b][V - 1], 1, 64);
            if (tx == 0 && active && i0 > 0) {
              Vec<T, 1> x1, x2, y1v, l1v, yn1, ln1;
              x1.v[0] = (a.x + pz - 1)[go]; x2.v[0] = xc.v[0];
              y1v.v[0] = (B.y + pz - 1)[go]; l1v.v[0] = (B.l + pz - 1)[go];
              const bool v1[1] = {true};
              T rp1[1], sv1[1];
              multi_block_update<T, 1, LK_X>(B, pc[b], x1, x2, v1, y1v, l1v, zerov<T, 1>(), yn1, ln1, rp1, sv1);
              lw = B.rho * yn1.v[0] + ln1.v[0];
              ld = yn1.v[0] - y1v.v[0];
            }
#pragma unroll
            for (int k = 0; k < V; ++k) {
              pw[k] = k == 0 ? lw : wv[b][k - 1];
              pd[k] = k == 0 ? ld : dv[b][k - 1];
              mm[k] = mxm[k];
              mc[k] = vx[k];
            }
          } else if constexpr (KIND == LK_Y) {
            constexpr int yi = lay_index_among(L, b, LK_Y);
            if (ty > 0) {
#pragma unroll
              for (int k = 0; k < V; ++k) { pw[k] = ybuf[par][yi][0][k][tid - LX]; pd[k] = ybuf[par][yi][1][k][tid - LX]; }
            } else {
#pragma unroll
              for (int k = 0; k < V; ++k) pw[k] = pd[k] = T(0);
              if (active && mym) {
                const Vec<T, V> x1 = ldv<T, V>(a.x + pz - st1 + go), yh = ldv<T, V>(B.y + pz - st1 + go), lh = ldv<T, V>(B.l + pz - st1 + go);
                Vec<T, V> yn, ln;
                bool valid[V];
#pragma unroll
                for (int k = 0; k < V; ++k) valid[k] = true;
                T rp1[V], sv1[V];
                multi_block_update<T, V, LK_Y>(B, pc[b], x1, xc, valid, yh, lh, zerov<T, V>(), yn, ln, rp1, sv1);
#pragma unroll
                for (int k = 0; k < V; ++k) { pw[k] = B.rho * yn.v[k] + ln.v[k]; pd[k] = yn.v[k] - yh.v[k]; }
              }
            }
#pragma unroll
            for (int k = 0; k < V; ++k) { mm[k] = mym; mc[k] = vy; }
          } else {
            constexpr int zi = lay_index_among(L, b, LK_Z);
#pragma unroll
            for (int k = 0; k < V; ++k) {
              pw[k] = zw[zi][k];
              pd[k] = zd[zi][k];
              mm[k] = mzm;
              mc[k] = vz;
              zw[zi][k] = wv[b][k];
              zd[zi][k] = dv[b][k];
            }
          }
          const T ih = B.ih, nih = -B.ih;
#pragma unroll
          for (int k = 0; k < V; ++k) {
            const T r1 = tr[k] + ih * pw[k];
            tr[k] = mm[k] ? r1 : tr[k];
            const T r2 = tr[k] + nih * wv[b][k];
            tr[k] = mc[k] ? r2 : tr[k];
            const T d1 = td[k] + ih * pd[k];
            td[k] = mm[k] ? d1 : td[k];
            const T d2 = td[k] + nih * dv[b][k];
            td[k] = mc[k] ? d2 : td[k];
          }
        }
        if constexpr (lay_last(L, b)) {
#pragma unroll
          for (int k = 0; k < V; ++k) {
            if (B.in_rhs) out[k] = out[k] + tr[k];
            if constexpr (KIND != LK_I && KIND != LK_D) { if (active && own) acc_du[b] += (double)td[k] * (double)td[k]; }
          }
        }
      });
      if (fuse_rhs && active && own) {
        Vec<T, V> o;
#pragma unroll
        for (int k = 0; k < V; ++k) o.v[k] = out[k];
        stv<T, V>(a.rhs + pz + go, o);
      }
    }
  }
  constexpr bool HAS_D = lay_count_kind(L, LK_D) > 0;
  constexpr int K0 = 2 * NSETS + (HAS_D ? 3 : 0);
  constexpr int K = K0 + (FULL ? NACC + 2 * NI : 0);
  double acc[K];
  int slots[K];
  {
    double rp_set = 0;
    static_for<0, NBLK>([&](auto bc) {
      constexpr int b = decltype(bc)::value;
      rp_set = lay_first(L, b) ? acc_rp[b] : rp_set + acc_rp[b];
      if constexpr (lay_last(L, b)) {
        constexpr int KIND = lay_kind(L, b);
        constexpr int si = lay_sets(L & ((1ull << (4 * b)) - 1ull));
        acc[2 * si] = rp_set;
        slots[2 * si] = a.b[b].set * SET_SLOTS + SL_RPRI;
        acc[2 * si + 1] = acc_du[b];
        slots[2 * si + 1] = a.b[b].set * SET_SLOTS + ((KIND == LK_I || KIND == LK_D) ? SL_DY : SL_ADJ);
        if constexpr (KIND == LK_D) {
          acc[2 * NSETS] = acc_obj; acc[2 * NSETS + 1] = acc_evo; acc[2 * NSETS + 2] = acc_xx;
          slots[2 * NSETS] = a.b[b].set * SET_SLOTS + SL_OBJ;
          slots[2 * NSETS + 1] = a.b[b].set * SET_SLOTS + SL_EVO;
          slots[2 * NSETS + 2] = a.b[b].set * SET_SLOTS + SL_XX;
        }
        if constexpr (FULL) {
#pragma unroll
          for (int q = 0; q < 6; ++q) {
            acc[K0 + 6 * si + q] = (tid & 3) == 0 ? lacc[6 * si + q][tid >> 2] : 0.0;
            slots[K0 + 6 * si + q] = a.b[b].set * SET_SLOTS + SL_HL + q;
          }
        }
      }
      if constexpr (FULL && lay_kind(L, b) == LK_I) {
        constexpr int ii = lay_index_among(L, b, LK_I);
        acc[K0 + 6 * NSETS + 2 * ii] = acc_fe[ii];
        acc[K0 + 6 * NSETS + 2 * ii + 1] = acc_ss[ii];
        slots[K0 + 6 * NSETS + 2 * ii] = a.b[b].set * SET_SLOTS + SL_FE;
        slots[K0 + 6 * NSETS + 2 * ii + 1] = a.b[b].set * SET_SLOTS + SL_SS;
      }
    });
  }
  __shared__ double sm[K][MULTI_NT / 64];
  const int lane = threadIdx.x & 63, w = threadIdx.x >> 6;
#pragma unroll
  for (int k = 0; k < K; ++k) {
    const double v = wave_sum(acc[k]);
    if (lane == 0) sm[k][w] = v;
  }
  __syncthreads();
  static_assert(K <= MULTI_NT, "one thread per slot in the epilogue");
  if (threadIdx.x < K) {
    double s = 0;
#pragma unroll
    for (int i = 0; i < MULTI_NT / 64; ++i) s += sm[threadIdx.x][i];
    int slot = slots[0];
#pragma unroll
    for (int k = 1; k < K; ++k) slot = (int)threadIdx.x == k ? slots[k] : slot;
    double* row = a.partials + (long long)slot * NB;
    row[blockIdx.x] = s;
    for (int jj = blockIdx.x + gridDim.x; jj < NB; jj += gridDim.x) row[jj] = 0.0;
  }
}

template <typename T, int V, unsigned long long L>
static void launch_multi(hipStream_t s, const Grid& g, const MultiArgs<T>& a, double bytes) {
  static_assert(SL_HH == SL_HL + 1 && SL_LH == SL_HL + 2 && SL_DL == SL_HL + 3 && SL_GG == SL_HL + 4 && SL_GL == SL_HL + 5, "BB slots");
  const long long nvx = g.n[0] / V;
  int lg = 0;
  while ((1 << lg) < nvx && lg < 6) ++lg;
  const int LX = 1 << lg, TY = MULTI_NT / LX;
  const bool three = g.n[1] > 1;
  const int xsplit = three ? 0 : 1;
  long long jlo = 0, jhi = g.n[1], jsum = 0, zlo = a.zlo, zhi = a.zhi;
  const bool empty = jhi <= jlo || zhi <= zlo;
  if (empty) { jhi = jlo + 1; zhi = zlo + 1; }
  const int tiles_x = xsplit ? (int)((nvx + (long long)LX * TY - 1) / ((long long)LX * TY)) : (int)((nvx + LX - 1) / LX);
  const int tiles_y = xsplit ? 1 : (int)((jhi - jlo + TY - 1) / TY);
  const long long tiles = (long long)tiles_x * tiles_y;
  const long long planes = zhi - zlo;
  const long long zc_env = env_knobs().multi_zchunk;
  long long want = (4ll * NB_7 + tiles - 1) / tiles;
  if (want < 1) want = 1;
  long long zchunk = (planes + want - 1) / want;
  if (zchunk < 8) zchunk = planes < 8 ? planes : 8;
  if (zc_env > 0) zchunk = zc_env < planes ? zc_env : planes;
  const long long nchunks = (planes + zchunk - 1) / zchunk;
  const long long items = empty ? 0 : tiles * nchunks;
  const int grid = (int)(items < 1 ? 1 : (items < NB_7 ? items : NB_7));
  MultiArgs<T> b = a;
  b.zlo = zlo; b.zhi = zhi;
  if (empty) { b.zlo = b.zhi = 0; }
  ObsScope obs(KID_YL_MULTI, s, bytes);
  if (a.flags && a.x0)
    hipLaunchKernelGGL((k_yl_multi<T, V, L, true, true>), dim3(grid), dim3(MULTI_NT), 0, s, g, b, lg, tiles_x, tiles_y, (int)zchunk, items, jlo, jhi, jsum, xsplit);
  else if (a.flags)
    hipLaunchKernelGGL((k_yl_multi<T, V, L, true, false>), dim3(grid), dim3(MULTI_NT), 0, s, g, b, lg, tiles_x, tiles_y, (int)zchunk, items, jlo, jhi, jsum, xsplit);
  else
    hipLaunchKernelGGL((k_yl_multi<T, V, L, false, false>), dim3(grid), dim3(MULTI_NT), 0, s, g, b, lg, tiles_x, tiles_y, (int)zchunk, items, jlo, jhi, jsum, xsplit);
  SIPX_HIP(hipGetLastError());
}

#define SIPX_LAYOUTS(F)                                                                                                          \
  F(lay_pack(lay_blk(LK_I, 1), lay_blk(LK_X, 1), lay_blk(LK_Y, 1), lay_blk(LK_Z, 1), lay_blk(LK_D, 1)))           \
  F(lay_pack(lay_blk(LK_I, 1), lay_blk(LK_Z, 0), lay_blk(LK_Y, 0), lay_blk(LK_X, 1), lay_blk(LK_D, 1)))         \
  F(lay_pack(lay_blk(LK_I, 1), lay_blk(LK_Z, 0), lay_blk(LK_X, 1), lay_blk(LK_D, 1)))                      \
  F(lay_pack(lay_blk(LK_I, 1), lay_blk(LK_X, 1), lay_blk(LK_Z, 1), lay_blk(LK_D, 1)))                                  \
  F(lay_pack(lay_blk(LK_I, 1), lay_blk(LK_Z, 1), lay_blk(LK_X, 1), lay_blk(LK_D, 1)))                      \
  F(lay_pack(lay_blk(LK_I, 1), lay_blk(LK_Z, 1), lay_blk(LK_D, 1)))                                                      \
  F(lay_pack(lay_blk(LK_I, 1), lay_blk(LK_Y, 1), lay_blk(LK_D, 1)))                                                      \
  F(lay_pack(lay_blk(LK_I, 1), lay_blk(LK_X, 1), lay_blk(LK_D, 1)))                                                      \
  F(lay_pack(lay_blk(LK_I, 1), lay_blk(LK_Z, 0), lay_blk(LK_Y, 0), lay_blk(LK_X, 1), lay_blk(LK_I, 1), lay_blk(LK_D, 1)))    \
  F(lay_pack(lay_blk(LK_I, 1), lay_blk(LK_D, 1)))                                                          \
  F(lay_pack(lay_blk(LK_I, 1), lay_blk(LK_X, 1), lay_blk(LK_Y, 1), lay_blk(LK_Z, 1), lay_blk(LK_I, 1), lay_blk(LK_D, 1)))

template <typename T>
bool K<T>::yl_multi(hipStream_t s, const Grid& g, const MultiArgs<T>& a, bool probe_only) {
  constexpr int V = sizeof(T) == 8 ? SIPX_MULTI_VF / 2 : SIPX_MULTI_VF;
  if (a.nblk < 1 || a.nblk > MULTI_MAXB || g.n[0] % V != 0) return false;
  unsigned long long code = 0;
  for (int b = 0; b < a.nblk; ++b) {
    const int px = a.b[b].prox;
    if (!(px == PX_BOUNDS || px == PX_L1 || px == PX_PROX_L1 || px == PX_L2 || px == PX_ANNULUS || px == PX_DIST)) return false;
    if (a.b[b].dir == 2 && g.n[2] <= 1) return false;
    const bool two_d = g.n[2] <= 1;
    const int kind = a.b[b].dist ? LK_D : (a.b[b].dir < 0 ? LK_I : (a.b[b].dir == 0 ? LK_X : (a.b[b].dir == 1 ? (two_d ? LK_Z : LK_Y) : LK_Z)));
    code |= lay_blk(kind, a.b[b].last != 0) << (4 * b);
  }
  const bool three = g.n[2] > 1;
  const double pts = (double)(a.zhi - a.zlo) * (three ? (double)g.st[2] : (double)g.st[1]);
  Grid gk = g;
  if (!three) {
    gk.n[1] = 1; gk.n[2] = g.n[1];
    gk.st[1] = g.n[0]; gk.st[2] = g.n[0];
  }
  double vecs = 1.0 + (a.rhs ? 1.0 : 0.0);
  const bool first = (a.flags & F_FIRST) != 0, bb = (a.flags & F_BB) != 0 && !first;
  const bool x0m = a.x0 != nullptr;
  for (int b = 0; b < a.nblk; ++b) vecs += 4.0 + (a.b[b].dist ? 2.0 : 0.0) + (bb ? (x0m ? 4.0 : 6.0) : (first ? (x0m ? 1.0 : 2.0) : 0.0));
  if (x0m) vecs += (bb ? 1.0 : 0.0) + ((a.x0w && (bb || first)) ? 1.0 : 0.0);
  const double bytes = vecs * pts * sizeof(T);
#define SIPX_TRY_LAYOUT(LL)                                    \
  if (code == (LL)) {                                          \
    if (!probe_only) launch_multi<T, V, (LL)>(s, gk, a, bytes); \
    return true;                                               \
  }
  SIPX_LAYOUTS(SIPX_TRY_LAYOUT)
#undef SIPX_TRY_LAYOUT
  return false;
}

template bool K<float>::yl_multi(hipStream_t, const Grid&, const MultiArgs<float>&, bool);
template bool K<double>::yl_multi(hipStream_t, const Grid&, const MultiArgs<double>&, bool);

}
```

setintersectionprojection.jl_amd/csrc/sipx_common.h:

```cpp
#pragma once
#include <hip/hip_runtime.h>
#include <stdint.h>
#include <cstdio>

#include "env_knobs.h"

namespace sipx {

constexpr int BLOCK = 256;
constexpr int NB = 2048;
constexpr int NB_7 = 1792;
inline int fit_grid(long long nvec, int cap) {
  const long long need = (nvec + BLOCK - 1) / BLOCK;
  return (int)(need < 1 ? 1 : (need < cap ? need : cap));
}
template <typename... P>
inline bool aligned16(const P*... p) {
  return (((reinterpret_cast<uintptr_t>(p) & 15u) == 0) && ...);
}
inline int launch_blocks(int per_cu) {
  static const int cus = [] {
    int dev = 0, n = 0;
    if (hipGetDevice(&dev) != hipSuccess || hipDeviceGetAttribute(&n, hipDeviceAttributeMultiprocessorCount, dev) != hipSuccess || n <= 0)
      n = 256;
    return n;
  }();
  const int g = per_cu * cus;
  return g < 256 ? 256 : (g > NB_7 ? NB_7 : g);
}
constexpr int MAXD = 32;
constexpr int MAX_SETS = 16;
constexpr int QT_N = 4 * 27;
constexpr int YL_SLOTS = 13;
constexpr int L1_K = 8;
#define SIPX_SOLVE_SLOTS 64
#define SIPX_MAX_WORLD 64
constexpr int GATHER_HDR = 8;
constexpr int PREP_SLOTS = 3 + 2 * L1_K;
template <typename T>
constexpr int fast_hdr() { return ((PREP_SLOTS + 4) * 8 / (int)sizeof(T) + 3) / 4 * 4; }
constexpr int SAMPLE_BINS = 1024;
constexpr int SAMPLE_MBITS = 7;

enum KernelId {
  KID_CDS_SPMV = 0, KID_CDS_DOT, KID_CDS_RESID, KID_CDS_FUSED, KID_SQ_SPMV, KID_SQ_DOT, KID_SQ_RESID, KID_CG_BEGIN, KID_CG_XR, KID_CG_P,
  KID_Q_UPDATE, KID_FIN_SUM, KID_RHS, KID_YL, KID_YL_MULTI, KID_ADJ_NORM, KID_LOG3, KID_PASS_FIRST, KID_PASS_LEAN, KID_PASS_PROBE,
  KID_PASS_COMPACT, KID_PASS_DIST, KID_PASS_STORE, KID_PASS_MULTI, KID_SLOT_SUMS, KID_DECIDE, KID_SAMPLE, KID_L1_SOLVE, KID_GATHER,
  KID_PS_RESCALE, KID_CARD, KID_EXT, KID_BB_RULE, KID_OTHER, KID_MF_FWD, KID_MF_ADJ, KID_L21_NORMS, KID_L21_FRAMES, KID_L21_SCALE,
  KID_L21J_NORMS, KID_L21J_FINISH, KID_L21J_SCALE, KID_L21W_PASS, KID_L21W_SCALE, KID_COUNT
};
inline const char* kernel_name(int k) {
  static const char* const names[KID_COUNT] = {
      "k_cds<MODE=0>", "k_cds<MODE=1>", "k_cds<MODE=2>", "k_cds_fused", "k_sq<MODE=0>", "k_sq<MODE=1>", "k_sq<MODE=2>", "k_cg_begin",
      "k_cg_update_xr", "k_cg_update_p", "k_q_update", "k_fin_sum", "k_rhs", "k_yl", "k_yl_multi", "k_adj_norm", "k_log3",
      "k_pass<M_FIRST>", "k_pass<M_LEAN>", "k_pass<M_PROBE>", "k_pass<M_COMPACT>", "k_pass<M_DIST>", "k_pass<M_STORE>", "k_pass_multi",
      "k_slot_sums", "k_decide", "k_sample", "k_l1_solve", "k_gather_pack/unpack", "k_ps_rescale", "k_card_*", "ext_proj (library-backed)",
      "k_bb_rule", "other", "k_mf_fwd", "k_mf_adj", "k_l21_norms", "k_l21_frames", "k_l21_scale",
      "k_l21j_norms", "k_l21j_finish", "k_l21j_scale", "k_l21w_part", "k_l21w_scale"};
  return (k >= 0 && k < KID_COUNT) ? names[k] : "?";
}
enum RouteId {
  RT_CDS_MARCH_BANDS = 0,
  RT_CDS_MARCH_TABLE = 4,
  RT_CDS_FLAT = 8,
  RT_CDS_FUSED_FLAT = 11,
  RT_RHS_MARCH = 12,
  RT_RHS_FLAT = 13,
  RT_COUNT = 14
};
inline const char* route_name(int r) {
  static const char* const names[RT_COUNT] = {
      "k_cds_march<MODE=0>/bands", "k_cds_march<MODE=1>/bands", "k_cds_march<MODE=2>/bands", "k_cds_march<MODE=3>/bands",
      "k_cds_march<MODE=0>/table", "k_cds_march<MODE=1>/table", "k_cds_march<MODE=2>/table", "k_cds_march<MODE=3>/table",
      "k_cds<MODE=0>", "k_cds<MODE=1>", "k_cds<MODE=2>", "k_cds_fused", "k_rhs_march", "k_rhs"};
  return (r >= 0 && r < RT_COUNT) ? names[r] : "?";
}
struct LaunchObserver {
  void* user;
  void (*begin)(void* user, int kid, hipStream_t s, double bytes_survey, double bytes_moved);
  void (*end)(void* user, int kid, hipStream_t s);
  void (*route)(void* user, int route);
};
const LaunchObserver*& launch_observer();

struct ObsScope {
  const LaunchObserver* o;
  int kid;
  hipStream_t s;
  ObsScope(int kid_, hipStream_t s_, double bytes_survey, double bytes_moved = -1.0) : o(launch_observer()), kid(kid_), s(s_) {
    if (env_knobs().trace_kernels) fprintf(stderr, "[sipx trace] %s\n", kernel_name(kid));
    if (o) o->begin(o->user, kid, s, bytes_survey, bytes_moved < 0 ? bytes_survey : bytes_moved);
  }
  ~ObsScope() {
    if (o) o->end(o->user, kid, s);
    if (env_knobs().trace_kernels) {
      (void)hipStreamSynchronize(s);
      fprintf(stderr, "[sipx trace]   done\n");
    }
  }
  void route(int r) const { if (o && o->route) o->route(o->user, r); }
  ObsScope(const ObsScope&) = delete;
  ObsScope& operator=(const ObsScope&) = delete;
};

enum { SL_RPRI = 0, SL_DY = 1, SL_HL = 2, SL_HH = 3, SL_LH = 4, SL_DL = 5, SL_GG = 6, SL_GL = 7,
       SL_FE = 8, SL_SS = 9, SL_OBJ = 10, SL_EVO = 11, SL_XX = 12,
       SL_ADJ = 13 , SL_FE2 = 14, SL_SS2 = 15  };
constexpr int SET_SLOTS = 16;

enum { F_FEAS = 1, F_BB = 2, F_FIRST = 4, F_NOSPEC = 8 ,
       F_STORE_DY = 16  };

enum { PX_BOUNDS = 0, PX_BOUNDS_VEC = 1, PX_L1 = 2, PX_L2 = 3, PX_ANNULUS = 4, PX_CARD = 5, PX_PROX_L1 = 6,
       PX_EXT = 8,
       PX_DIST = 100 };

struct Grid {
  long long n[3];
  long long N;
  long long st[3];
  unsigned m1 = 0, s1 = 0, m2 = 0, s2 = 0;
  long long e0 = 0, e1 = -1, s0 = 0;
  void set_fast_div() {
    auto magic = [](long long d, unsigned& m, unsigned& sh) {
      m = 0; sh = 0;
      if (d < 2 || d >= (1ll << 31)) return;
      int l = 0;
      while ((1ll << l) < d) ++l;
      const unsigned long long q = ((unsigned long long)1 << (31 + l)) / (unsigned long long)d + 1ull;
      m = (unsigned)q;
      sh = (unsigned)(l - 1);
    };
    magic(n[0], m1, s1);
    magic(n[1], m2, s2);
  }
};

inline long long range_len(const Grid& g) { return (g.e1 < 0 ? g.N : g.e1) - g.e0; }

struct CdsArgs {
  int d;
  long long off[MAXD];
  int sym = 0;
  int partner[MAXD] = {};
  int march = 0;
  int mb[4] = {0, 0, 0, 0};
  long long gn[3] = {0, 0, 0};
  const void* qtab = nullptr;
};

template <typename T>
struct StencilQ {
  T w0, w[3];
  int mask;
};

template <typename T>
// ... 109 lines not shown
struct SpecFinishSet {
  ProjScalars<T>* ps;
  DecideArgs da;
  double* reg;
  const T* fseg0;
  T* compact;
  const double* partials;
  T radius;
  int* host_want;
  unsigned* verdict;
};
template <typename T>
struct SpecFinishArgs {
  int local = 0;
  int nsets, world;
  long long fchunk;
  unsigned seq;
  SpecFinishSet<T> s[SPEC_MAX_SETS];
};

template <typename T>
struct SampleSet {
  SetArgs<T> a;
  ProjScalars<T>* ps;
  double* partials;
  double* reg;
  long long true_len;
};
template <typename T>
struct SampleMulti {
  int v_is_s = 0;
  int ns;
  SampleSet<T> s[SPEC_MAX_SETS];
};
template <typename T>
struct RescaleMulti {
  int n;
  ProjScalars<T>* ps[SPEC_MAX_SETS];
  double factor[SPEC_MAX_SETS];
};

template <typename T>
struct LeanSet {
  SetArgs<T> a;
  ProjScalars<T>* ps;
  T* compact;
  double* partials;
  T* maxpart;
};
constexpr int LEAN_MAX = 3;
template <typename T>
struct LeanMulti {
  int v_is_s = 0;
  int ns;
  LeanSet<T> s[LEAN_MAX];
};

constexpr int MULTI_MAXB = 8;
template <typename T>
struct MultiBlk {
  const T *y, *l;
  T *yo, *lo;
  T *lh0, *s0;
  const T *y0, *l0;
  const ProjScalars<T>* ps;
  int dir;
  int set;
  int first, last;
  int dist;
  int feas_el;
  int in_rhs = 1;
  T ih, rho, rho1, gamma;
  int prox;
  T plo, phi;
};
template <typename T>
struct MultiArgs {
  int nblk;
  MultiBlk<T> b[MULTI_MAXB];
  const T *x, *m, *xold;
  const T* x0;
  T* x0w;
  T* rhs;
  double* partials;
  int flags;
  long long zlo, zhi;
  long long zsum;
};

template <typename T>
struct MkSet {
  T alpha;
  int nblk, comp;
  int dir[3];
  T ih[3];
};
template <typename T>
struct MkArgs {
  int nsets;
  MkSet<T> s[MAX_SETS];
};

template <typename T>
struct QSet {
  T alpha;
  const T* ata;
  int nblk;
  int dir[3];
  T ih[3];
  int nband;
  long long off[9];
};
template <typename T>
struct QArgs {
  int nsets;
  QSet<T> s[MAX_SETS];
};

template <typename T>
struct RhsSet {
  const T *y, *l;
  T rho;
  int nblk;
  int dir[3];
  T ih[3];
};
template <typename T>
struct RhsArgs {
  int nsets;
  RhsSet<T> s[MAX_SETS];
};

template <typename T>
struct MfOp {
  int rows = 0;
  long long nnz = 0;
  const int* ptr = nullptr;
  const int* idx = nullptr;
  const T* val = nullptr;
  int lanes = 1;
};
template <typename T>
struct MfAdj {
  const T *y = nullptr, *l = nullptr;
  T rho = T(0), alpha = T(1);
  T* out = nullptr;
  const T* p = nullptr;
  double* partials = nullptr;
  int in_mode = 0, dot = 0, slot = 0;
  const int* done = nullptr;
};

template <typename T>
struct CgState {
  double ss;
  T rr;
  T gamma, alpha, beta;
  T nr0, tol, res_last;
  int done, flag, iters;
  T tol_ref;
  int it_outer;
  unsigned seq;
};

template <typename T>
struct K {
  static void spmv(hipStream_t s, const Grid& g, long long N, const T* R, const CdsArgs& a, const T* x, T* y);
  static void spmv_dot(hipStream_t s, long long N, long long r0, long long r1, const T* R, const CdsArgs& a, const T* p, T* Ap,
                       double* partials, const CgState<T>* st);
  static void resid(hipStream_t s, long long N, long long r0, long long r1, const T* R, const CdsArgs& a, const T* x, const T* b,
                    T* r, T* p, T* xold, double* partials);
  static void spmv_fused(hipStream_t s, long long N, const T* R, const CdsArgs& a, const T* r, const T* p_old, T* p_new, T* Ap,
                         double* partials, CgState<T>* st, CgState<T>* host, unsigned long long* ticket);
  static void sq_spmv(hipStream_t s, const Grid& g, const StencilQ<T>& q, const T* x, T* y);
  static void sq_spmv_dot(hipStream_t s, const Grid& g, const StencilQ<T>& q, const T* p, T* Ap, double* partials,
                          const CgState<T>* st);
  static void sq_resid(hipStream_t s, const Grid& g, const StencilQ<T>& q, const T* x, const T* b, T* r, T* p, T* xold,
                       double* partials);
  static void q_axpy(hipStream_t s, long long N, T* Qband, const T* Aband, T alpha);
  static void q_update(hipStream_t s, const Grid& g, long long r0, long long r1, const CdsArgs& q, const QArgs<T>& a, T* Q);
  static void gen_ata(hipStream_t s, const Grid& g, int nblk, const int* dir, const T* ih, int nband,
                      const long long* offs, T* R);
  static void cg_begin(hipStream_t s, double* partials, CgState<T>* st, CgState<T>* host, int it_outer, T tol_ref,
                       unsigned seq, unsigned long long* ticket);
  static void cg_update_xr(hipStream_t s, long long N, const T* x_in, T* x, const T* r_in, T* r, const T* p, const T* Ap, double* partials,
                           CgState<T>* st, CgState<T>* host, int iter, unsigned long long* ticket, long long hlo = 0,
                           long long hhi = 0);
  static void cg_update_p(hipStream_t s, long long N, T* p, const T* r, const double* partials, CgState<T>* st,
                          CgState<T>* host, unsigned long long* ticket, long long hlo = 0, long long hhi = 0);
  static void rhs_compose(hipStream_t s, const Grid& g, const RhsArgs<T>& a, T* rhs, int accumulate);
  static void yl(hipStream_t s, const Grid& g, const SetArgs<T>& a, double* partials);
  static void adj_norm(hipStream_t s, const Grid& g, const SetArgs<T>& a, double* partials);
  static bool yl_multi(hipStream_t s, const Grid& g, const MultiArgs<T>& a, bool probe_only = false);
  static void fwd(hipStream_t s, const Grid& g, int nblk, const int* dir, const T* ih, const T* x, T* out);
  static void adj(hipStream_t s, const Grid& g, int nblk, const int* dir, const T* ih, const T* v, T* out);
  static void log3(hipStream_t s, long long N, const T* x, const T* m, const T* xold, double* partials);
  static void q_update_mk(hipStream_t s, const Grid& g, const CdsArgs& q, const MkArgs<T>& a, T* Q);
  static void mirror_bands(hipStream_t s, long long N, const CdsArgs& q, T* Q);
  static bool march_applies(long long N, const CdsArgs& a);
  static void qtab_build(hipStream_t s, long long N, const CdsArgs& q, const T* Q, T* tab, int* ok);
  static bool qtab_update(hipStream_t s, const Grid& g, const CdsArgs& q, const QArgs<T>& a, T* tab);
  static void qtab_write_bands(hipStream_t s, long long N, const CdsArgs& q, const T* tab, T* Q);
  static void sum_uv(hipStream_t s, long long N, const T* u, const T* v, T* w);
  static void csr_spmv(hipStream_t s, long long M, const long long* rowptr, const long long* col, const T* val, const T* x, T* out);
  static void csc_adj_rhs(hipStream_t s, long long N, const long long* colptr, const long long* row, const T* val, const T* y,
                          const T* l, T rho, T* out, int accumulate);
  static void csc_adj_norm(hipStream_t s, long long N, const long long* colptr, const long long* row, const T* val, const T* dy,
                           double* partials);
  static void mf_fwd(hipStream_t s, const MfOp<T>& A, const T* x, T* out, const int* done);
  static void mf_adj(hipStream_t s, const MfOp<T>& At, const MfAdj<T>& a);
  static void rows_pack(hipStream_t s, const Grid& g, int dir, long long nrows, const T* pad, T* rows);
  static void rows_unpack(hipStream_t s, const Grid& g, int dir, long long nrows, const T* rows, T* pad);
  static void fin_sum(hipStream_t s, const double* partials, int nslots, double* out_dev, double* out_host, unsigned* ticket = nullptr,
                      unsigned long long* word = nullptr, unsigned long long seq = 0);
  static void copy_f64(hipStream_t s, const double* src, double* dst, int n);
  static void ps_rescale(hipStream_t s, ProjScalars<T>* ps, double factor);
  static void proj_scalars_set(hipStream_t s, const Grid& g, const SetArgs<T>& a, int v_is_s, ProjScalars<T>* ps,
                               double* partials, T* maxpart, T* compact, long long true_len, SampleCtl ctl = SampleCtl(),
                               const ChainHooks* hooks = nullptr);
  static void spec_sums_pack(hipStream_t s, const SpecPackArgs<T>& A);
  static void spec_finish(hipStream_t s, SpecFinishArgs<T>& A);
  static void ps_rescale_multi(hipStream_t s, const RescaleMulti<T>& A);
  static void sample_multi(int stage, hipStream_t s, const Grid& g, const SampleMulti<T>& A, long long runs, const ChainHooks* hk);
  static void lean_multi(hipStream_t s, const Grid& g, const LeanMulti<T>& m);
  static void pass_multi(int mode, hipStream_t s, const Grid& g, const LeanMulti<T>& m, int v_is_s);
  static void search_tail(int stage, hipStream_t s, const SetArgs<T>& a, ProjScalars<T>* ps, double* partials, T* maxpart, T* compact,
                          long long true_len, SampleCtl ctl, double* reg);
  static void proj_scalars_stage(int stage, hipStream_t s, const Grid& g, const SetArgs<T>& a, int v_is_s, ProjScalars<T>* ps,
                                 double* partials, T* maxpart, T* compact, long long true_len, SampleCtl ctl, const ChainHooks* hooks,
                                 double* reg, T* gseg0, long long chunk);
  static void proj_scalars_arr(hipStream_t s, long long len, const T* v, int prox, T pmin, T pmax, ProjScalars<T>* ps,
                               double* partials, T* maxpart, T* compact, long long true_len);
  static void proj_scalars_arr_slab(hipStream_t s, long long len, const T* v, int prox, T pmin, T pmax, ProjScalars<T>* ps,
                                    double* partials, T* maxpart, T* compact, long long true_len, const ChainHooks* hooks,
                                    long long compact_len, int* host_ovf);
  static void proj_dist_set(hipStream_t s, const Grid& g, const SetArgs<T>& a, int v_is_s, const ProjScalars<T>* ps,
                            double* dst);
  static void ps_init(hipStream_t s, ProjScalars<T>* ps, long long* cidx);
  static void store_v(hipStream_t s, const Grid& g, const SetArgs<T>& a, int v_is_s, T* out);
};

template <typename T>
void proj_dist_grid(hipStream_t s, const Grid& g, int nblk, const int* dir, long long len, const T* v, int prox, T plo,
                    T phi, const T* lb, const T* ub, const ProjScalars<T>* ps, double* partials);
template <typename T>
void proj_apply_grid(hipStream_t s, const Grid& g, int nblk, const int* dir, long long len, T* v, int prox, T plo,
                     T phi, const T* lb, const T* ub, const ProjScalars<T>* ps);

template <typename T>
void prox_l2s_dev(hipStream_t s, long long n, T* x, const T* m, T rho);

template <typename T>
void resample_nn(hipStream_t s, const long long* nc, const long long* nf, const T* in, T* out);
template <typename T>
void resample_nn_rows(hipStream_t s, const long long* nc, const long long* nf, int nblk, const int* dir, int b, long long cstride,
                      long long e0, long long e1, const T* in, T* out);
template <typename T>
void resample_nn_padded(hipStream_t s, const long long* nc, const long long* nf, const long long* cc, const long long* cf, long long e0,
                        long long e1, const T* in, T* out);

constexpr int IO_MAXSEG = 32;
template <typename T>
struct IoSeg {
  T* rows;
  T* pad;
  unsigned nrows, d0, d1, n0, n1, blk0, linear, vec, bdir;
};
template <typename T>
struct IoArgs {
  int nseg = 0;
  unsigned nblocks = 0;
  IoSeg<T> seg[IO_MAXSEG];
};
template <typename T>
void io_seg_shape(IoSeg<T>& S, const Grid& g, int dir, long long nrows, const T* rows, const T* pad);
template <typename T>
// ... 12 lines not shown
```

setintersectionprojection.jl_amd/csrc/sipx_device.h:

```cpp
#pragma once
#include "sipx_common.h"

namespace sipx {

template <typename T, int V>
struct alignas(sizeof(T) * V) Vec {
  T v[V];
};

template <typename T, int V>
__device__ __forceinline__ Vec<T, V> ldv(const T* p) {
  return *reinterpret_cast<const Vec<T, V>*>(p);
}
template <typename T, int V>
__device__ __forceinline__ void stv(T* p, const Vec<T, V>& x) {
  *reinterpret_cast<Vec<T, V>*>(p) = x;
}
template <typename T, int V>
__device__ __forceinline__ Vec<T, V> ldv_nt(const T* p) {
  typedef T vt __attribute__((ext_vector_type(V)));
  Vec<T, V> r;
  if constexpr (V == 1) {
    r.v[0] = __builtin_nontemporal_load(p);
  } else if constexpr (sizeof(T) * V == 16) {
// ... 217 lines not shown
    }
  }
  __device__ __forceinline__ void add_lean(T av, int k_lo, int k_hi) {
    const double a = (double)av;
    asum += a;
#pragma unroll
    for (int k = 0; k < L1_K; ++k) {
      if (k != k_lo && k != k_hi) continue;
      const bool on = av > t[k];
      S[k] += on ? a : 0.0;
      C[k] += on ? 1u : 0u;
    }
  }
  __device__ __forceinline__ void to_slots(double (&acc)[PREP_SLOTS]) const {
    acc[0] = asum; acc[1] = sumsq; acc[2] = (double)nnz;
#pragma unroll
    for (int k = 0; k < L1_K; ++k) { acc[3 + k] = S[k]; acc[3 + L1_K + k] = (double)C[k]; }
  }
};

template <typename T>
__device__ __forceinline__ T eps_of();
template <>
__device__ __forceinline__ float eps_of<float>() { return 1.1920928955078125e-07f; }
template <>
__device__ __forceinline__ double eps_of<double>() { return 2.220446049250313e-16; }

__device__ __forceinline__ double jl_max(double a, double b) { return (a != a || b != b) ? (a + b) : (a > b ? a : b); }
__device__ __forceinline__ double jl_min(double a, double b) { return (a != a || b != b) ? (a + b) : (a < b ? a : b); }

struct Coord {
  int i, j, k;
};
template <int V>
__device__ __forceinline__ void vec_range(const Grid& G, long long& v0, long long& v1) {
  v0 = G.e0 / V;
  v1 = (G.e1 < 0 ? G.N : G.e1) / V;
}
__device__ __forceinline__ Coord coords(const Grid& G, long long g) {
  Coord c;
  const unsigned u = (unsigned)g, n1 = (unsigned)G.n[0], n2 = (unsigned)G.n[1];
  const unsigned jk = G.m1 ? (__umulhi(u, G.m1) >> G.s1) : u / n1;
  c.i = (int)(u - jk * n1);
  const unsigned k = G.m2 ? (__umulhi(jk, G.m2) >> G.s2) : jk / n2;
  c.j = (int)(jk - k * n2);
  c.k = (int)k;
  return c;
}
__device__ __forceinline__ int coord_of(const Coord& c, int dir) { return dir == 0 ? c.i : (dir == 1 ? c.j : c.k); }

template <typename T, int V>
__device__ __forceinline__ void fwd_dir(const Grid& G, const T* __restrict__ x, const Vec<T, V>& xc, long long g,
                                        const Coord& c, int dir, T ih, T (&s)[V], bool (&valid)[V]) {
  const T nih = -ih;
  const long long st = dir == 0 ? 1 : (dir == 1 ? G.st[1] : G.st[2]);
  const int nd = (int)(dir == 0 ? G.n[0] : (dir == 1 ? G.n[1] : G.n[2]));
  const int cd = coord_of(c, dir);
  const Vec<T, V> xn = ldv_u<T, V>(x + g + st);
#pragma unroll
  for (int k = 0; k < V; ++k) {
    valid[k] = (cd + (dir == 0 ? k : 0)) < nd - 1;
    const T d = nih * xc.v[k] + ih * xn.v[k];
    s[k] = valid[k] ? d : T(0);
  }
}

template <typename T, int V, typename WV>
__device__ __forceinline__ void adj_dir_acc(const Grid& G, long long g, const Coord& c, int dir, T ih, T (&t)[V],
                                            WV wv) {
  const T nih = -ih;
  const long long st = dir == 0 ? 1 : (dir == 1 ? G.st[1] : G.st[2]);
  const int nd = (int)(dir == 0 ? G.n[0] : (dir == 1 ? G.n[1] : G.n[2]));
  const int cd = coord_of(c, dir);
  const Vec<T, V> wc = wv(g);
  const Vec<T, V> wp = wv(g - st);
#pragma unroll
  for (int k = 0; k < V; ++k) {
    const int ck = cd + (dir == 0 ? k : 0);
    const T t1 = t[k] + ih * wp.v[k];
    t[k] = (ck > 0) ? t1 : t[k];
    const T t2 = t[k] + nih * wc.v[k];
    t[k] = (ck < nd - 1) ? t2 : t[k];
  }
}

template <typename T>
__device__ __forceinline__ T soft_thr(T v, T th) {
  T t = fabs(v) - th;
  t = t > T(0) ? t : T(0);
  return v > T(0) ? t : (v < T(0) ? -t : v);
}

template <typename T>
struct ProxCtx {
  int prox;
  T plo, phi, rho, theta, scale, tau;
  int fill;
  long long idx_cut;
};

template <typename T>
__device__ __forceinline__ ProxCtx<T> make_prox(int prox, T plo, T phi, T rho, const ProjScalars<T>* ps) {
  ProxCtx<T> c;
  c.prox = prox;
  c.plo = plo;
  c.phi = phi;
  c.rho = rho;
  c.theta = T(0);
  c.scale = T(1);
  c.tau = T(0);
  c.fill = 0;
  c.idx_cut = -1;
  if (ps) {
    c.theta = ps->theta;
    c.scale = ps->scale;
    c.fill = ps->fill;
    c.tau = ps->tau;
    c.idx_cut = ps->quota;
  }
  if (prox == PX_PROX_L1) c.theta = T(1) / phi;
  return c;
}

template <typename T>
__device__ __forceinline__ T prox_apply(const ProxCtx<T>& c, T v, T lb, T ub, T m, long long e) {
  switch (c.prox) {
    case PX_BOUNDS: {
      T t = v < c.phi ? v : c.phi;
      return c.plo > t ? c.plo : t;
    }
    case PX_BOUNDS_VEC: {
      if (c.plo != T(0)) {
        T t = v > lb ? v : lb;
        return t < ub ? t : ub;
      }
      T t = v < ub ? v : ub;
      return lb > t ? lb : t;
    }
    case PX_DIST:
      return (T)((double)(v * c.rho + m) / ((double)c.rho + 1.0));
    case PX_L1:
    case PX_PROX_L1:
      return soft_thr(v, c.theta);
    case PX_L2:
    case PX_ANNULUS:
      return c.fill ? c.scale : v * c.scale;
    case PX_CARD: {
      const T av = fabs(v);
      return (av > c.tau || (av == c.tau && e <= c.idx_cut)) ? v : T(0);
    }
  }
  return v;
}


}
```

setintersectionprojection.jl_amd/host.py:

```python
from __future__ import annotations

import ctypes as C
import os
from dataclasses import dataclass, field
from typing import Any, List, Optional, Sequence, Tuple

import numpy as np

LIB_PATH = os.environ.get("SIPX_LIBRARY") or os.path.join(os.path.dirname(os.path.abspath(__file__)), "libsipx.so")

EXPORTED_SYMBOLS = [
    "sipx_last_error", "sipx_create", "sipx_destroy", "sipx_add_set", "sipx_set_rows", "sipx_num_terms",
    "sipx_finalize", "sipx_rhs_compose", "sipx_argmin_x", "sipx_update_y_l", "sipx_log_scalars",
    "sipx_adapt_rho_gamma", "sipx_q_update", "sipx_download", "sipx_parsdmm", "sipx_parsdmm_begin",
    "sipx_parsdmm_steps", "sipx_cds_spmv",
    "sipx_apply_op", "sipx_apply_op_adj", "sipx_project", "sipx_get_Q", "sipx_time_spmv", "sipx_kernel_stats",
    "sipx_debug_proj", "sipx_resample_nn", "sipx_set_q_mode", "sipx_apply_Q",
    "sipx_stream",
    "sipx_dev_rhs", "sipx_dev_x", "sipx_set_owned", "sipx_get_rhs", "sipx_prox_l2s",
    "sipx_rccl_unique_id", "sipx_set_comm_rccl", "sipx_set_comm", "sipx_slab", "sipx_warm_start_from", "sipx_set_decomp",
    "sipx_kernel_stats_json", "sipx_comm_info", "sipx_device_bytes", "sipx_reset", "sipx_dwt",
    "sipx_learn_observations",
    "sipx_finalize_dev", "sipx_reset_dev", "sipx_download_dev", "sipx_set_caller_stream", "sipx_io_bytes",
    "sipx_q_terms", "sipx_set_data", "sipx_set_data_dev", "sipx_segment_norms", "sipx_segment_norms_dev",
    "sipx_l21_norm", "sipx_l21_norm_dev", "sipx_l21_norms", "sipx_l21_norms_dev",
    "sipx_l21_joint_norm", "sipx_l21_joint_norm_dev", "sipx_l21_weighted_norm", "sipx_l21_weighted_norm_dev",
]

SIPX_F32, SIPX_F64 = 0, 1
OPS = {"identity": 0, "D_x": 1, "D_y": 2, "D_z": 3, "TV": 4, "D2D": 4, "D3D": 4, "custom": 5, "TV_xy": 6}
PROJ = {"bounds": 0, "bounds_vec": 1, "l1": 2, "l2": 3, "annulus": 4, "cardinality": 5, "prox_l1": 6, "l1_dft": 7, "rank": 8,
        "nuclear": 9, "histogram": 10, "subspace": 11, "bounds_dft": 12, "card_dft": 13, "l21": 14, "l21_joint": 15}
TV_OPERATORS = ("TV", "D2D", "D3D")
L21_NEEDS_TV = "the l2,1 ball acts on the range of the TV operator: TD_OP must be TV (D2D, D3D)"
L21_WHOLE_ONLY = "the l2,1 ball applies to the whole array (mode matrix/tensor)"
L21_FRAMES_Z = "the l2,1 ball on TV_xy: frames run along z -- the mode must be (slice, z), or tensor for the whole array"
L21_JOINT_NEEDS_TV_XY = "the joint l2,1 ball groups the frames of TV_xy: TD_OP must be TV_xy, mode tensor"
L21_WEIGHTS_WHERE = ("weights belong to the l2,1 sets on the whole array -- (\"l21\", \"TV\"), (\"l21\", \"TV_xy\") in tensor mode and "
                     "(\"l21_joint\", \"TV_xy\"): drop them, or use one of these sets")
L21_WEIGHTS_NO_FRAMES = ("the l2,1 ball per frame takes no weights: use (\"l21\", \"TV_xy\") in tensor mode or (\"l21_joint\", \"TV_xy\"), "
                         "which take one weight per group")
L21_WEIGHTS_NO_COARSE = ("multilevel: a weighted l2,1 set has no rule that takes its weights to a coarser grid yet -- solve on one level, "
                         "or drop the weights")
UNKNOWN_OPERATOR = "provided an unknown transform domain operator. check function get_TD_operator(comp_grid,TD_type,TF) for options"
TV_XY_NEEDS_3D = UNKNOWN_OPERATOR + " (TV_xy is the in-plane gradient of a 3-D grid; on a 2-D grid TV is in-plane already)"
TV_XY_NO_MINKOWSKI = "the TV_xy operator takes no Minkowski component"
TV_XY_NO_MULTILEVEL = "the TV_xy operator is not built for PARSDMM_multi_level: solve on one level"
MODES = {"matrix": 0, "tensor": 0, "fiber": 1, "slice": 2}
TRANSFORMS = {"DCT": 1, "wavelet": 2}
SPECIAL_OPERATORS = ("DFT", "DCT", "wavelet", "curvelet")
YL_FEAS, YL_BB, YL_FIRST = 1, 2, 4
Q_MODES = {"cds": 0, "stencil": 1}
MAX_Q_BANDS = 32


class SipxError(RuntimeError):
    pass


class _SetDesc(C.Structure):
    _fields_ = [("op", C.c_int32), ("proj", C.c_int32), ("pmin", C.c_double), ("pmax", C.c_double),
                ("lb", C.c_void_p), ("ub", C.c_void_p), ("ncvx", C.c_int32), ("reserved", C.c_int32),
                ("mode", C.c_int32), ("dir", C.c_int32), ("basis", C.c_void_p), ("basis_rows", C.c_int64),
                ("basis_cols", C.c_int32), ("basis_orth", C.c_int32), ("component", C.c_int32),
                ("csc_colptr", C.c_void_p), ("csc_rowval", C.c_void_p), ("csc_nzval", C.c_void_p), ("csc_rows", C.c_int64),
                ("transform", C.c_int32), ("pad_", C.c_int32)]


class _Options(C.Structure):
    _fields_ = [("maxit", C.c_int32), ("evol_rel_tol", C.c_double), ("feas_tol", C.c_double),
                ("obj_tol", C.c_double), ("rho_update_frequency", C.c_int32), ("adjust_rho", C.c_int32),
                ("adjust_gamma", C.c_int32), ("adjust_feasibility_rho", C.c_int32)]


class _Log(C.Structure):
    _fields_ = [(k, C.c_void_p) for k in ("set_feasibility", "r_dual", "r_pri", "r_dual_total", "r_pri_total",
                                           "obj", "evol_x", "rho", "gamma", "cg_it", "cg_relres")] + \
               [("timing_ms", C.c_double * 7), ("n_iter", C.c_int32), ("n_feas_rows", C.c_int32),
                ("stopped_feasible", C.c_int32)]


_lib = None
_default_device = 0


def set_default_device(device: int):
    global _default_device
    _default_device = int(device)


def lib():
    global _lib
    if _lib is None:
        if not os.path.exists(LIB_PATH):
            raise SipxError(f"{LIB_PATH} is missing -- run `python -c 'import __graft_entry__ as g; g.build()'`; "
                            "the engine has no CPU fallback")
        L = C.CDLL(LIB_PATH)
        L.sipx_last_error.restype = C.c_char_p
        for name in ("sipx_stream", "sipx_dev_rhs", "sipx_dev_x"):
            getattr(L, name).restype = C.c_void_p
            getattr(L, name).argtypes = [C.c_void_p]
        L.sipx_kernel_stats_json.restype = C.c_char_p
# ... 846 lines not shown
        return a.value, b.value

    def finalize_dev(self, m, rho_ini, gamma_ini, feasibility_only=False, zero_ini_guess=True, x0=None, l0=None, y0=None):
        return self._start(True, False, m, rho_ini, gamma_ini, feasibility_only, zero_ini_guess, x0, l0, y0)

    def reset_dev(self, m, rho_ini, gamma_ini, zero_ini_guess=True, x0=None, l0=None, y0=None):
        return self._start(True, True, m, rho_ini, gamma_ini, False, zero_ini_guess, x0, l0, y0)

    def download_dev(self, device, want_ly=True, out=None):
        import torch
        dt = torch.float32 if self.TF == np.float32 else torch.float64
        ox, ol, oy = (None, None, None) if out is None else out
        if ox is None:
            ox = torch.empty(self.Nx, dtype=dt, device=device)
        else:
            _check_tensor("out x", ox, self.TF, self.Nx, device)
        res = [ox]
        for name, lst in (("out l", ol), ("out y", oy)):
            if not want_ly:
                res.append(None)
            elif lst is None:
                res.append([torch.empty(r, dtype=dt, device=device) for r in self.rows])
            else:
                _check_tensor_list(name, lst, self.TF, self.rows, device)
                res.append(lst)
        x, l, y = res
        self.set_caller_stream(torch.cuda.current_stream(device).cuda_stream)
        _chk(lib().sipx_download_dev(self.h, _tensor_ptr(x), _ptr_array(l, _tensor_ptr), _ptr_array(y, _tensor_ptr)))
        return x, l, y

    def rhs_compose(self, rho):
        rho = np.ascontiguousarray(rho, np.float64)
        _chk(lib().sipx_rhs_compose(self.h, _ptr(rho)))

    def argmin_x(self, it, tol_ref):
        t, ci, rr, fl = C.c_double(tol_ref), C.c_int64(), C.c_double(), C.c_int()
        _chk(lib().sipx_argmin_x(self.h, int(it), C.byref(t), C.byref(ci), C.byref(rr), C.byref(fl)))
        return t.value, ci.value, rr.value, fl.value

    def update_y_l(self, it, flags, rho, gamma):
        rho = np.ascontiguousarray(rho, np.float64); gamma = np.ascontiguousarray(gamma, np.float64)
        rp, rd, fe = np.zeros(self.p), np.zeros(self.p), np.zeros(max(self.pp, 1))
        _chk(lib().sipx_update_y_l(self.h, int(it), int(flags), _ptr(rho), _ptr(gamma), _ptr(rp), _ptr(rd), _ptr(fe)))
        return rp, rd, fe[:self.pp]

    def log_scalars(self):
        a, b = C.c_double(), C.c_double()
        _chk(lib().sipx_log_scalars(self.h, C.byref(a), C.byref(b)))
        return a.value, b.value

    def adapt_rho_gamma(self, adjust_rho, adjust_gamma, rho, gamma):
        rho = np.array(rho, np.float64); gamma = np.array(gamma, np.float64)
        _chk(lib().sipx_adapt_rho_gamma(self.h, int(adjust_rho), int(adjust_gamma), _ptr(rho), _ptr(gamma)))
        return rho, gamma

    def q_update(self, rho_new, rho_old):
        a = np.ascontiguousarray(rho_new, np.float64); b = np.ascontiguousarray(rho_old, np.float64)
        _chk(lib().sipx_q_update(self.h, _ptr(a), _ptr(b)))

    def download(self, want_ly=True, x_out=None):
        if (x_out is not None and isinstance(x_out, np.ndarray) and x_out.dtype == self.TF and x_out.shape == (self.Nx,)
                and x_out.flags.c_contiguous and x_out.flags.writeable):
            x = x_out
        else:
            x = np.empty(self.Nx, self.TF)
        l = [np.zeros(r, self.TF) for r in self.rows] if want_ly else None
        y = [np.zeros(r, self.TF) for r in self.rows] if want_ly else None
        _chk(lib().sipx_download(self.h, _ptr(x), _ptr_array(l), _ptr_array(y)))
        return x, l, y

    def warm_start_from(self, coarse: "Context"):
        _chk(lib().sipx_warm_start_from(self.h, coarse.h))

    def slab(self):
        a, b, c = C.c_int64(), C.c_int64(), C.c_int64()
        _chk(lib().sipx_slab(self.h, C.byref(a), C.byref(b), C.byref(c)))
        return a.value, b.value, c.value

    def get_rhs(self):
        rhs = np.empty(self.Nx, self.TF)
        _chk(lib().sipx_get_rhs(self.h, _ptr(rhs)))
        return rhs

    def get_Q(self):
        d = C.c_int()
        offs = np.zeros(32, np.int64)
        _chk(lib().sipx_get_Q(self.h, None, _ptr(offs), C.byref(d)))
        Q = np.empty((self.Nx, d.value), self.TF, order="F")
        _chk(lib().sipx_get_Q(self.h, _ptr(Q), _ptr(offs), C.byref(d)))
        return Q, offs[:d.value].copy()

    def time_spmv(self, reps=20):
        ms = C.c_double()
        _chk(lib().sipx_time_spmv(self.h, int(reps), C.byref(ms)))
        return ms.value

    def debug_proj(self, set_index: int, which: int = 0):
        out = np.zeros(16)
        _chk(lib().sipx_debug_proj(self.h, int(set_index), int(which), _ptr(out)))
        keys = ("need", "theta", "theta_prev", "hw", "spec_lo", "spec_hi", "lo", "hi", "asum", "vmax", "gathered",
                "overflow", "spec_ok", "michelot_its", "refine", "lean")
        d = dict(zip(keys, out))
        d["sampled"] = float(int(d["lean"]) >> 1)
        d["lean"] = float(int(d["lean"]) & 1)
        return d

    def kernel_stats(self, enable):
        n, ms = C.c_int64(), C.c_double()
        _chk(lib().sipx_kernel_stats(self.h, int(enable), C.byref(n), C.byref(ms)))
        return n.value, ms.value

    def kernel_stats_all(self, enable):
        import json
        txt = lib().sipx_kernel_stats_json(self.h, int(enable))
        if txt is None:
            raise SipxError(lib().sipx_last_error().decode())
        return json.loads(txt.decode())

    def device_bytes(self):
        a, b, c = C.c_int64(), C.c_int64(), C.c_int64()
        _chk(lib().sipx_device_bytes(self.h, C.byref(a), C.byref(b), C.byref(c)))
        return {"context": a.value, "device_used": b.value, "device_total": c.value}

    def comm_info(self):
        n, r, d = C.c_int(), C.c_int(), C.c_int()
        ver = C.create_string_buffer(64)
        _chk(lib().sipx_comm_info(self.h, C.byref(n), C.byref(r), ver, 64, C.byref(d)))
        return {"nranks": n.value, "rank": r.value, "version": ver.value.decode(), "decomposition": "slab" if d.value == 1 else "sets"}

    def _log_struct(self, options: PARSDMM_options):
        maxit, p, pp = int(options.maxit), self.p, self.pp
        o = _Options(maxit, float(options.evol_rel_tol), float(options.feas_tol), float(options.obj_tol),
                     int(options.rho_update_frequency), int(options.adjust_rho), int(options.adjust_gamma),
                     int(options.adjust_feasibility_rho))
        arrs = dict(set_feasibility=np.zeros((maxit, max(pp, 1))), r_dual=np.zeros((maxit, p)),
                    r_pri=np.zeros((maxit, p)), r_dual_total=np.zeros(maxit), r_pri_total=np.zeros(maxit),
                    obj=np.zeros(maxit), evol_x=np.zeros(maxit), rho=np.zeros((maxit, p)),
                    gamma=np.zeros((maxit, p)), cg_it=np.zeros(maxit, np.int64), cg_relres=np.zeros(maxit))
        lg = _Log()
        for k, a in arrs.items():
            setattr(lg, k, a.ctypes.data)
        return o, lg, arrs

    def _log_result(self, lg, arrs):
        it, nf, pp = lg.n_iter, lg.n_feas_rows, self.pp
        return log_type_PARSDMM(arrs["set_feasibility"][:nf, :pp], arrs["r_dual"][:it], arrs["r_pri"][:it],
                                arrs["r_dual_total"][:it], arrs["r_pri_total"][:it], arrs["obj"][:it],
                                arrs["evol_x"][:it], arrs["rho"][:it], arrs["gamma"][:it], arrs["cg_it"][:it],
                                arrs["cg_relres"][:it],
                                dict(zip(TIMING_SECTIONS, [t * 1e-3 for t in lg.timing_ms])))

    def parsdmm(self, options: PARSDMM_options):
        o, lg, arrs = self._log_struct(options)
        _chk(lib().sipx_parsdmm(self.h, C.byref(o), C.byref(lg)))
        return self._log_result(lg, arrs), bool(lg.stopped_feasible)

    def parsdmm_begin(self, options: PARSDMM_options):
        self._run = self._log_struct(options)
        o, lg, arrs = self._run
        _chk(lib().sipx_parsdmm_begin(self.h, C.byref(o), C.byref(lg)))

    def parsdmm_steps(self, nsteps: int) -> bool:
        done = C.c_int()
        _chk(lib().sipx_parsdmm_steps(self.h, int(nsteps), C.byref(done)))
        return bool(done.value)

# ... 662 lines not shown
```

Measured before the change: 891.8.

## Form the CG initial residual inside the fused y/l sweep and defer rhs

The fused y/l multi-block sweep gains a variant that also computes the 7-point Q·x product from a shared-memory coefficient table. It writes the initial CG residual r0 = rhs - Qx together with its norm partials, so the x-step head (separate SpMV and rhs pass) can be skipped. The rhs itself is marked stale and rebuilt only when a caller asks for it. The variant is enabled only for f32 on a single device with the table-driven march path, and by default only on grids above 2^24 points. The aim is to remove a full extra pass over x and rhs per iteration, at the cost of more registers and boundary logic in the sweep kernel.

Measured after the change: 880.8. 1.2% lower.

```diff
diff --git a/include/sipx.h b/include/sipx.h
--- a/include/sipx.h
+++ b/include/sipx.h
@@ -166,6 +166,7 @@
 void* sipx_dev_rhs(sipx_ctx* ctx);
 void* sipx_dev_x(sipx_ctx* ctx);
 int sipx_get_rhs(sipx_ctx* ctx, void* rhs);
+int sipx_get_r0(sipx_ctx* ctx, void* r0);
 int sipx_prox_l2s(int dtype, int64_t n, void* x, double rho, const void* m, int device);
 int sipx_set_owned(sipx_ctx* ctx, const int32_t* owned);
 
diff --git a/setintersectionprojection.jl_amd/csrc/api.cpp b/setintersectionprojection.jl_amd/csrc/api.cpp
--- a/setintersectionprojection.jl_amd/csrc/api.cpp
+++ b/setintersectionprojection.jl_amd/csrc/api.cpp
@@ -181,6 +181,7 @@
 void* sipx_dev_rhs(sipx_ctx* c) { return c->e->dev_rhs(); }
 void* sipx_dev_x(sipx_ctx* c) { return c->e->dev_x(); }
 int sipx_get_rhs(sipx_ctx* c, void* rhs) { SIPX_TRY(c->e->get_rhs(rhs)) }
+int sipx_get_r0(sipx_ctx* c, void* r0) { SIPX_TRY(c->e->get_r0(r0)) }
 int sipx_prox_l2s(int dtype, int64_t n, void* x, double rho, const void* m, int device) {
   SIPX_TRY(sipx::refresh_env_knobs(); sipx::prox_l2s_host(dtype, n, x, rho, m, device))
 }
diff --git a/setintersectionprojection.jl_amd/csrc/engine.cpp b/setintersectionprojection.jl_amd/csrc/engine.cpp
--- a/setintersectionprojection.jl_amd/csrc/engine.cpp
+++ b/setintersectionprojection.jl_amd/csrc/engine.cpp
@@ -851,7 +851,7 @@
     batch_searches_ = batch_fallbacks_ = 0;
     for (long long& c : routes_) c = 0;
     head_done_ = false; rs_pending_ = false; sums_pending_ = false; merged_nslots_ = 0;
-    rhs_fused_ = false; have_log_sums_ = false;
+    rhs_fused_ = false; have_log_sums_ = false; rhs_stale_ = false;
     obj_ss_ = evo_ss_ = xx_ss_ = 0;
     sums_flags_ = 0;
     marks_.reset();
@@ -933,6 +933,7 @@
     need_final();
     ObserverGuard og(observer());
     head_done_ = false;
+    rhs_stale_ = false;
     if (rs_pending_) {
       SIPX_HIP(hipStreamWaitEvent(stream_, ev_c_[1], 0));
       rs_pending_ = false;
@@ -950,6 +951,17 @@
       }
       return;
     }
+    rhs_launches(rho);
+    if (comm_ && !slab_) {
+      SIPX_HIP(hipEventRecord(ev_c_[0], stream_));
+      SIPX_HIP(hipStreamWaitEvent(cstream_, ev_c_[0], 0));
+      comm_->reduce_scatter_sum(rhs_, (size_t)chunk_, dtype_code(), cstream_);
+      SIPX_HIP(hipEventRecord(ev_c_[1], cstream_));
+      rs_pending_ = true;
+    }
+  }
+
+  void rhs_launches(const double* rho) {
     RhsBatch b(stream_, Gr_, rhs_, false);
     for (int i = 0; i < p_n_; ++i)
       if (sets_[i].owned && !sets_[i].custom) b.add(sets_[i], (T)rho[i]);
@@ -959,16 +971,16 @@
       const SetState<T>& s = sets_[i];
       if (s.owned && s.custom) custom_adj_rhs(stream_, s, (T)rho[i]);
     }
-    if (comm_ && !slab_) {
-      SIPX_HIP(hipEventRecord(ev_c_[0], stream_));
-      SIPX_HIP(hipStreamWaitEvent(cstream_, ev_c_[0], 0));
-      comm_->reduce_scatter_sum(rhs_, (size_t)chunk_, dtype_code(), cstream_);
-      SIPX_HIP(hipEventRecord(ev_c_[1], cstream_));
-      rs_pending_ = true;
-    }
+  }
+  void ensure_rhs() {
+    if (!rhs_stale_) return;
+    ObserverGuard og(observer());
+    rhs_launches(rhs_rho_.data());
+    rhs_stale_ = false;
   }
 
   void argmin_x_head() {
+    ensure_rhs();
     if (rs_pending_) {
       SIPX_HIP(hipStreamWaitEvent(stream_, ev_c_[1], 0));
       rs_pending_ = false;
@@ -2099,8 +2111,21 @@
     ma.x0w = nullptr;
     ma.rhs = fuse_rhs ? rhs_ : nullptr;
     ma.partials = part_sets_;
+    ma.r0 = nullptr;
+    if (fuse_rhs && cds_.qtab && cg_fused_ && !has_loose_ && !slab_ && !comm_ && n_mfree_ == 0 &&
+        (G_.N > (1ll << 24) || env_knobs().cds_march == 2)) {
+      ma.r0 = p_; ma.part_cg = part_cg_; ma.qtab = (const T*)cds_.qtab; ma.qord = cds_.march;
+    }
+    const bool forms_r0 = K<T>::yl_multi_forms_r0(G_, ma);
     if (!K<T>::yl_multi(stream_, G_, ma)) throw std::runtime_error("internal: the fused y/l sweep refused a block list it was prepared for");
     rhs_fused_ = ma.rhs != nullptr;
+    if (forms_r0) {
+      head_done_ = true;
+      rhs_stale_ = true;
+      rhs_rho_.assign(rho, rho + p_n_);
+    } else if (rhs_fused_) {
+      rhs_stale_ = false;
+    }
     if (x0_mode_ && (first || bb)) x_snap_ = x_cur_;
     for (int i = 0; i < p_n_; ++i) {
       SetState<T>& s = sets_[i];
@@ -2697,6 +2722,7 @@
     }
     if (!R.rhs_ready) return;
     marks_.open(i + 1);
+    if (head_done_) return;
     argmin_x_head();
     if (comm_) {
       marks_.mark(-1);
@@ -3168,13 +3194,24 @@
   }
 
   void* stream() override { return (void*)stream_; }
-  void* dev_rhs() override { return rhs_; }
+  void* dev_rhs() override {
+    ensure_rhs();
+    return rhs_;
+  }
   void* dev_x() override { return x_; }
   void get_rhs(void* out) override {
     need_final();
     if (slab_local_ && comm_->world > 1) throw std::runtime_error("a slab-decomposed context holds its planes of rhs only");
+    ensure_rhs();
     SIPX_HIP(hipStreamSynchronize(stream_));
     SIPX_HIP(hipMemcpy(out, rhs_, Nx_ * sizeof(T), hipMemcpyDeviceToHost));
+  }
+  void get_r0(void* out) override {
+    need_final();
+    if (!head_done_) throw std::runtime_error("no residual formed ahead of an x-step is pending");
+    if (comm_) throw std::runtime_error("sipx_get_r0: one rank only");
+    SIPX_HIP(hipStreamSynchronize(stream_));
+    SIPX_HIP(hipMemcpy(out, p_, Nx_ * sizeof(T), hipMemcpyDeviceToHost));
   }
 
  private:
@@ -3843,6 +3880,8 @@
   DeviceMemory mem_;
   bool slab_dist_logs_ = false;
   bool lean_multi_ = false;
+  bool rhs_stale_ = false;
+  std::vector<double> rhs_rho_;
   bool head_done_ = false;
   int merged_nslots_ = 0;
   int sums_flags_ = 0;
diff --git a/setintersectionprojection.jl_amd/csrc/engine.h b/setintersectionprojection.jl_amd/csrc/engine.h
--- a/setintersectionprojection.jl_amd/csrc/engine.h
+++ b/setintersectionprojection.jl_amd/csrc/engine.h
@@ -58,6 +58,7 @@
   virtual void* dev_rhs() = 0;
   virtual void* dev_x() = 0;
   virtual void get_rhs(void* out) = 0;
+  virtual void get_r0(void* out) = 0;
   virtual void set_owned(const int32_t* owned) = 0;
   virtual void set_q_mode(int mode) = 0;
   virtual void set_decomp(int mode) = 0;
diff --git a/setintersectionprojection.jl_amd/csrc/kernels_cds.hip b/setintersectionprojection.jl_amd/csrc/kernels_cds.hip
--- a/setintersectionprojection.jl_amd/csrc/kernels_cds.hip
+++ b/setintersectionprojection.jl_amd/csrc/kernels_cds.hip
@@ -122,10 +122,6 @@
   }
 }
 
-constexpr int march_role(int ord, int b) {
-  constexpr int o1[7] = {0, 1, 2, 3, 4, 5, 6}, o2[7] = {0, 5, 3, 1, 2, 4, 6};
-  return ord == 1 ? o1[b] : o2[b];
-}
 template <typename T>
 __device__ __forceinline__ T ata_value(const Grid& G, int nblk, const int* dir, const T* ihs, long long o, const Coord& c) {
   T val = (nblk == 0 && o == 0) ? T(1) : T(0);
@@ -177,16 +173,6 @@
 }
 template <typename X, typename T>
 __device__ __forceinline__ void load_class_tab(const X&, T*) {}
-__device__ __forceinline__ int line_class(long long c, long long n) { return c == 0 ? 0 : (c == n - 1 ? 2 : 1); }
-template <typename T, int V>
-__device__ __forceinline__ Vec<T, V> tab_row(const T* tab, int role, int cyz, long long i0, long long n1) {
-  const T* e = tab + 27 * role + cyz;
-  const T first = e[0], mid = e[1], last = e[2];
-  Vec<T, V> v;
-#pragma unroll
-  for (int k = 0; k < V; ++k) v.v[k] = i0 + k == 0 ? first : (i0 + k == n1 - 1 ? last : mid);
-  return v;
-}
 __device__ __forceinline__ void publish_ticket(unsigned long long* ticket, unsigned seq, int iter, int done);
 constexpr int MARCH_NT = 512;
 template <typename T, int V, int ORD, int MODE, typename X>
diff --git a/setintersectionprojection.jl_amd/csrc/kernels_multi.hip b/setintersectionprojection.jl_amd/csrc/kernels_multi.hip
--- a/setintersectionprojection.jl_amd/csrc/kernels_multi.hip
+++ b/setintersectionprojection.jl_amd/csrc/kernels_multi.hip
@@ -47,6 +47,12 @@
   int n = 0;
   for (int b = 0; b < MULTI_MAXB; ++b) n += (lay_kind(L, b) != 0 && lay_last(L, b)) ? 1 : 0;
   return n;
+}
+constexpr int lay_r0_ord(unsigned long long L) {
+  if (L == lay_pack(lay_blk(LK_I, 1), lay_blk(LK_X, 1), lay_blk(LK_Y, 1), lay_blk(LK_Z, 1), lay_blk(LK_D, 1))) return 1;
+  if (L == lay_pack(lay_blk(LK_I, 1), lay_blk(LK_Z, 0), lay_blk(LK_Y, 0), lay_blk(LK_X, 1), lay_blk(LK_D, 1))) return 2;
+  if (L == lay_pack(lay_blk(LK_I, 1), lay_blk(LK_Z, 0), lay_blk(LK_Y, 0), lay_blk(LK_X, 1), lay_blk(LK_I, 1), lay_blk(LK_D, 1))) return 2;
+  return 0;
 }
 
 template <typename T>
@@ -108,7 +114,7 @@
   }
 }
 
-template <typename T, int V, unsigned long long L, bool FULL, bool X0>
+template <typename T, int V, unsigned long long L, bool FULL, bool X0, int RORD = 0>
 __global__ __launch_bounds__(MULTI_NT, SIPX_MULTI_WAVES) void k_yl_multi(Grid G, MultiArgs<T> a, int lgLX, int tiles_x, int tiles_y, int zchunk,
                                                        long long items, long long jlo, long long jhi, long long jsum, int xsplit) {
   constexpr int NBLK = lay_count(L), NY = lay_count_kind(L, LK_Y), NZ = lay_count_kind(L, LK_Z);
@@ -116,6 +122,14 @@
   constexpr int NACC = FULL ? 6 * NSETS : 1;
   __shared__ double lacc[NACC][MULTI_NT / 4];
   __shared__ T ybuf[2][NY > 0 ? NY : 1][2][V][MULTI_NT];
+  constexpr bool R0 = RORD != 0;
+  static_assert(!R0 || (!FULL && NY > 0 && lay_count_kind(L, LK_X) > 0 && NZ > 0), "the residual form: plain variant, all seven bands");
+  __shared__ T ctab[R0 ? QT_N : 1];
+  if constexpr (R0) {
+    for (int i = threadIdx.x; i < QT_N; i += MULTI_NT) ctab[i] = a.qtab[i];
+    __syncthreads();
+  }
+  double acc_r0 = 0, acc_bb = 0;
   const bool f_first = FULL && (a.flags & F_FIRST) != 0, f_bb = FULL && (a.flags & F_BB) != 0 && !f_first;
   const bool f_feas = FULL && (a.flags & F_FEAS) != 0;
   if constexpr (FULL) {
@@ -177,6 +191,7 @@
     });
 
     Vec<T, V> xnext = active ? ldv<T, V>(a.x + st2 * k0 + go) : zerov<T, V>();
+    Vec<T, V> xprev = (R0 && active) ? ldv<T, V>(a.x + st2 * (k0 - 1) + go) : zerov<T, V>();
     constexpr bool x0mode = FULL && X0;
     Vec<T, V> x0next = (x0mode && f_bb && active) ? ldv<T, V>(a.x0 + st2 * k0 + go) : zerov<T, V>();
     for (long long kz = k0; kz < k1; ++kz) {
@@ -185,7 +200,8 @@
       const Vec<T, V> xc = xnext;
       const bool vz = kz < n3 - 1, mzm = kz > 0;
       const bool own = kz >= a.zsum && j >= jsum;
-      Vec<T, V> xpx = zerov<T, V>(), xpy = zerov<T, V>();
+      Vec<T, V> xpx = zerov<T, V>(), xpy = zerov<T, V>(), xup = zerov<T, V>();
+      T xl = T(0);
       Vec<T, V> yv[NBLK], lv[NBLK], mv = zerov<T, V>(), xo = zerov<T, V>();
 #pragma unroll
       for (int b = 0; b < NBLK; ++b) { yv[b] = zerov<T, V>(); lv[b] = zerov<T, V>(); }
@@ -193,6 +209,10 @@
         xnext = ldv_u<T, V>(a.x + pz + st2 + go);
         if constexpr (lay_count_kind(L, LK_X) > 0) xpx = ldv_u<T, V>(a.x + pz + 1 + go);
         if constexpr (NY > 0) xpy = ldv_u<T, V>(a.x + pz + st1 + go);
+        if constexpr (R0) {
+          xup = ldv<T, V>(a.x + pz - st1 + go);
+          if (tx == 0 || (tid & 63) == 0) xl = (a.x + pz - 1)[go];
+        }
         if constexpr (SIPX_MULTI_PREFETCH && !FULL) {
 #pragma unroll
           for (int b = 0; b < NBLK; ++b) {
@@ -210,6 +230,68 @@
           if constexpr (NY > 0) x0py = ldv_u<T, V>(a.x0 + pz + st1 + go);
         }
         if (x0mode && a.x0w && (f_bb || f_first) && active) stv_nt<T, V>(a.x0w + pz + go, xc);
+      }
+      T qx[R0 ? V : 1];
+      if constexpr (R0) {
+#pragma unroll
+        for (int k = 0; k < V; ++k) qx[k] = T(0);
+        const T sl = __shfl_up(xc.v[V - 1], 1, 64);
+        if (!(tx == 0 || (tid & 63) == 0)) xl = sl;
+        if (active) {
+          const long long r = pz + go, N = st2 * n3;
+          const long long i0g = i0;
+          const int cy = line_class(j, n2), cz = line_class(kz, n3), cyz = 3 * cy + 9 * cz;
+          const int cyz_up = j > 0 ? 3 * line_class(j - 1, n2) + 9 * cz : 3 * line_class(n2 - 1, n2) + 9 * line_class(kz - 1, n3);
+          const bool up = r >= st1, down = r + st1 < N, below = r >= st2, above = r + st2 < N, first = r == 0, last = r + V == N;
+#pragma unroll
+          for (int q = 0; q < 7; ++q) {
+            const int role = march_role(RORD, q);
+            Vec<T, V> rv = zerov<T, V>(), xv = zerov<T, V>();
+            bool in[V];
+            if (role == 0) {
+              rv = tab_row<T, V>(ctab, 0, cyz, i0g, n1);
+              xv = xc;
+#pragma unroll
+              for (int k = 0; k < V; ++k) in[k] = true;
+            } else if (role == 1) {
+              const Vec<T, V> r1 = tab_row<T, V>(ctab, 1, cyz, i0g, n1);
+              T rl = T(0);
+              if (r > 0) rl = i0g > 0 ? ctab[27 + line_class(i0g - 1, n1) + cyz] : ctab[27 + line_class(n1 - 1, n1) + cyz_up];
+#pragma unroll
+              for (int k = 0; k < V; ++k) { rv.v[k] = k == 0 ? rl : r1.v[k - 1]; xv.v[k] = k == 0 ? xl : xc.v[k - 1]; in[k] = k > 0 || !first; }
+            } else if (role == 2) {
+              rv = tab_row<T, V>(ctab, 1, cyz, i0g, n1);
+#pragma unroll
+              for (int k = 0; k < V; ++k) { xv.v[k] = xpx.v[k]; in[k] = k < V - 1 || !last; }
+            } else if (role == 3) {
+              if (r - st1 >= 0) rv = tab_row<T, V>(ctab, 2, cyz_up, i0g, n1);
+              xv = xup;
+#pragma unroll
+              for (int k = 0; k < V; ++k) in[k] = up;
+            } else if (role == 4) {
+              rv = tab_row<T, V>(ctab, 2, cyz, i0g, n1);
+              xv = xpy;
+#pragma unroll
+              for (int k = 0; k < V; ++k) in[k] = down;
+            } else if (role == 5) {
+              if (kz > 0) rv = tab_row<T, V>(ctab, 3, 3 * cy + 9 * line_class(kz - 1, n3), i0g, n1);
+              xv = xprev;
+#pragma unroll
+              for (int k = 0; k < V; ++k) in[k] = below;
+            } else {
+              rv = tab_row<T, V>(ctab, 3, cyz, i0g, n1);
+              xv = xnext;
+#pragma unroll
+              for (int k = 0; k < V; ++k) in[k] = above;
+            }
+#pragma unroll
+            for (int k = 0; k < V; ++k) {
+              const T t = qx[k] + rv.v[k] * xv.v[k];
+              qx[k] = in[k] ? t : qx[k];
+            }
+          }
+        }
+        xprev = xc;
       }
       T wv[NBLK][V], dv[NBLK][V];
       static_for<0, NBLK>([&](auto bc) {
@@ -416,7 +498,18 @@
           }
         }
       });
-      if (fuse_rhs && active && own) {
+      if constexpr (R0) {
+        if (active && own) {
+          Vec<T, V> o;
+#pragma unroll
+          for (int k = 0; k < V; ++k) {
+            o.v[k] = out[k] - qx[k];
+            acc_r0 += (double)o.v[k] * (double)o.v[k];
+            acc_bb += (double)out[k] * (double)out[k];
+          }
+          stv<T, V>(a.r0 + pz + go, o);
+        }
+      } else if (fuse_rhs && active && own) {
         Vec<T, V> o;
 #pragma unroll
         for (int k = 0; k < V; ++k) o.v[k] = out[k];
@@ -426,9 +519,13 @@
   }
   constexpr bool HAS_D = lay_count_kind(L, LK_D) > 0;
   constexpr int K0 = 2 * NSETS + (HAS_D ? 3 : 0);
-  constexpr int K = K0 + (FULL ? NACC + 2 * NI : 0);
+  constexpr int K = K0 + (FULL ? NACC + 2 * NI : 0) + (R0 ? 2 : 0);
   double acc[K];
   int slots[K];
+  if constexpr (R0) {
+    acc[K - 2] = acc_r0; slots[K - 2] = -1;
+    acc[K - 1] = acc_bb; slots[K - 1] = -2;
+  }
   {
     double rp_set = 0;
     static_for<0, NBLK>([&](auto bc) {
@@ -480,7 +577,7 @@
     int slot = slots[0];
 #pragma unroll
     for (int k = 1; k < K; ++k) slot = (int)threadIdx.x == k ? slots[k] : slot;
-    double* row = a.partials + (long long)slot * NB;
+    double* row = (R0 && slot < 0) ? a.part_cg + (long long)(-1 - slot) * NB : a.partials + (long long)slot * NB;
     row[blockIdx.x] = s;
     for (int jj = blockIdx.x + gridDim.x; jj < NB; jj += gridDim.x) row[jj] = 0.0;
   }
@@ -515,6 +612,15 @@
   b.zlo = zlo; b.zhi = zhi;
   if (empty) { b.zlo = b.zhi = 0; }
   ObsScope obs(KID_YL_MULTI, s, bytes);
+  constexpr int RORD = sizeof(T) == 4 ? lay_r0_ord(L) : 0;
+  if constexpr (RORD != 0) {
+    if (a.r0) {
+      obs.route(RT_YL_MULTI_R0);
+      hipLaunchKernelGGL((k_yl_multi<T, V, L, false, false, RORD>), dim3(grid), dim3(MULTI_NT), 0, s, g, b, lg, tiles_x, tiles_y, (int)zchunk, items, jlo, jhi, jsum, xsplit);
+      SIPX_HIP(hipGetLastError());
+      return;
+    }
+  }
   if (a.flags && a.x0)
     hipLaunchKernelGGL((k_yl_multi<T, V, L, true, true>), dim3(grid), dim3(MULTI_NT), 0, s, g, b, lg, tiles_x, tiles_y, (int)zchunk, items, jlo, jhi, jsum, xsplit);
   else if (a.flags)
@@ -538,8 +644,27 @@
   F(lay_pack(lay_blk(LK_I, 1), lay_blk(LK_X, 1), lay_blk(LK_Y, 1), lay_blk(LK_Z, 1), lay_blk(LK_I, 1), lay_blk(LK_D, 1)))
 
 template <typename T>
-bool K<T>::yl_multi(hipStream_t s, const Grid& g, const MultiArgs<T>& a, bool probe_only) {
+bool K<T>::yl_multi_forms_r0(const Grid& g, const MultiArgs<T>& a) {
+  if (sizeof(T) != 4 || !a.r0 || !a.rhs || !a.qtab || !a.part_cg || a.flags || g.n[2] <= 1) return false;
+  if (a.zlo != 0 || a.zhi != g.n[2] || a.zsum != 0) return false;
+  unsigned long long code = 0;
+  for (int b = 0; b < a.nblk && b < MULTI_MAXB; ++b) {
+    if (!a.b[b].in_rhs) return false;
+    const int kind = a.b[b].dist ? LK_D : (a.b[b].dir < 0 ? LK_I : (a.b[b].dir == 0 ? LK_X : (a.b[b].dir == 1 ? LK_Y : LK_Z)));
+    code |= lay_blk(kind, a.b[b].last != 0) << (4 * b);
+  }
+  int ord = 0;
+#define SIPX_R0_LAYOUT(LL) if (code == (LL)) ord = lay_r0_ord(LL);
+  SIPX_LAYOUTS(SIPX_R0_LAYOUT)
+#undef SIPX_R0_LAYOUT
+  return ord != 0 && ord == a.qord;
+}
+
+template <typename T>
+bool K<T>::yl_multi(hipStream_t s, const Grid& g, const MultiArgs<T>& a0, bool probe_only) {
   constexpr int V = sizeof(T) == 8 ? SIPX_MULTI_VF / 2 : SIPX_MULTI_VF;
+  MultiArgs<T> a = a0;
+  if (!yl_multi_forms_r0(g, a)) a.r0 = nullptr;
   if (a.nblk < 1 || a.nblk > MULTI_MAXB || g.n[0] % V != 0) return false;
   unsigned long long code = 0;
   for (int b = 0; b < a.nblk; ++b) {
@@ -573,6 +698,8 @@
   return false;
 }
 
+template bool K<float>::yl_multi_forms_r0(const Grid&, const MultiArgs<float>&);
+template bool K<double>::yl_multi_forms_r0(const Grid&, const MultiArgs<double>&);
 template bool K<float>::yl_multi(hipStream_t, const Grid&, const MultiArgs<float>&, bool);
 template bool K<double>::yl_multi(hipStream_t, const Grid&, const MultiArgs<double>&, bool);
 
diff --git a/setintersectionprojection.jl_amd/csrc/sipx_common.h b/setintersectionprojection.jl_amd/csrc/sipx_common.h
--- a/setintersectionprojection.jl_amd/csrc/sipx_common.h
+++ b/setintersectionprojection.jl_amd/csrc/sipx_common.h
@@ -66,13 +66,14 @@
   RT_CDS_FUSED_FLAT = 11,
   RT_RHS_MARCH = 12,
   RT_RHS_FLAT = 13,
-  RT_COUNT = 14
+  RT_YL_MULTI_R0 = 14,
+  RT_COUNT = 15
 };
 inline const char* route_name(int r) {
   static const char* const names[RT_COUNT] = {
       "k_cds_march<MODE=0>/bands", "k_cds_march<MODE=1>/bands", "k_cds_march<MODE=2>/bands", "k_cds_march<MODE=3>/bands",
       "k_cds_march<MODE=0>/table", "k_cds_march<MODE=1>/table", "k_cds_march<MODE=2>/table", "k_cds_march<MODE=3>/table",
-      "k_cds<MODE=0>", "k_cds<MODE=1>", "k_cds<MODE=2>", "k_cds_fused", "k_rhs_march", "k_rhs"};
+      "k_cds<MODE=0>", "k_cds<MODE=1>", "k_cds<MODE=2>", "k_cds_fused", "k_rhs_march", "k_rhs", "k_yl_multi/r0"};
   return (r >= 0 && r < RT_COUNT) ? names[r] : "?";
 }
 struct LaunchObserver {
@@ -348,6 +349,10 @@
   const T* x0;
   T* x0w;
   T* rhs;
+  T* r0 = nullptr;
+  double* part_cg = nullptr;
+  const T* qtab = nullptr;
+  int qord = 0;
   double* partials;
   int flags;
   long long zlo, zhi;
@@ -458,6 +463,7 @@
   static void yl(hipStream_t s, const Grid& g, const SetArgs<T>& a, double* partials);
   static void adj_norm(hipStream_t s, const Grid& g, const SetArgs<T>& a, double* partials);
   static bool yl_multi(hipStream_t s, const Grid& g, const MultiArgs<T>& a, bool probe_only = false);
+  static bool yl_multi_forms_r0(const Grid& g, const MultiArgs<T>& a);
   static void fwd(hipStream_t s, const Grid& g, int nblk, const int* dir, const T* ih, const T* x, T* out);
   static void adj(hipStream_t s, const Grid& g, int nblk, const int* dir, const T* ih, const T* v, T* out);
   static void log3(hipStream_t s, long long N, const T* x, const T* m, const T* xold, double* partials);
diff --git a/setintersectionprojection.jl_amd/csrc/sipx_device.h b/setintersectionprojection.jl_amd/csrc/sipx_device.h
--- a/setintersectionprojection.jl_amd/csrc/sipx_device.h
+++ b/setintersectionprojection.jl_amd/csrc/sipx_device.h
@@ -323,6 +323,21 @@
     const T t2 = t[k] + nih * wc.v[k];
     t[k] = (ck < nd - 1) ? t2 : t[k];
   }
+}
+
+constexpr int march_role(int ord, int b) {
+  constexpr int o1[7] = {0, 1, 2, 3, 4, 5, 6}, o2[7] = {0, 5, 3, 1, 2, 4, 6};
+  return ord == 1 ? o1[b] : o2[b];
+}
+__device__ __forceinline__ int line_class(long long c, long long n) { return c == 0 ? 0 : (c == n - 1 ? 2 : 1); }
+template <typename T, int V>
+__device__ __forceinline__ Vec<T, V> tab_row(const T* tab, int role, int cyz, long long i0, long long n1) {
+  const T* e = tab + 27 * role + cyz;
+  const T first = e[0], mid = e[1], last = e[2];
+  Vec<T, V> v;
+#pragma unroll
+  for (int k = 0; k < V; ++k) v.v[k] = i0 + k == 0 ? first : (i0 + k == n1 - 1 ? last : mid);
+  return v;
 }
 
 template <typename T>
diff --git a/setintersectionprojection.jl_amd/host.py b/setintersectionprojection.jl_amd/host.py
--- a/setintersectionprojection.jl_amd/host.py
+++ b/setintersectionprojection.jl_amd/host.py
@@ -17,7 +17,7 @@
     "sipx_apply_op", "sipx_apply_op_adj", "sipx_project", "sipx_get_Q", "sipx_time_spmv", "sipx_kernel_stats",
     "sipx_debug_proj", "sipx_resample_nn", "sipx_set_q_mode", "sipx_apply_Q",
     "sipx_stream",
-    "sipx_dev_rhs", "sipx_dev_x", "sipx_set_owned", "sipx_get_rhs", "sipx_prox_l2s",
+    "sipx_dev_rhs", "sipx_dev_x", "sipx_set_owned", "sipx_get_rhs", "sipx_get_r0", "sipx_prox_l2s",
     "sipx_rccl_unique_id", "sipx_set_comm_rccl", "sipx_set_comm", "sipx_slab", "sipx_warm_start_from", "sipx_set_decomp",
     "sipx_kernel_stats_json", "sipx_comm_info", "sipx_device_bytes", "sipx_reset", "sipx_dwt",
     "sipx_learn_observations",
@@ -1030,6 +1030,11 @@
         _chk(lib().sipx_get_rhs(self.h, _ptr(rhs)))
         return rhs
 
+    def get_r0(self):
+        r0 = np.empty(self.Nx, self.TF)
+        _chk(lib().sipx_get_r0(self.h, _ptr(r0)))
+        return r0
+
     def get_Q(self):
         d = C.c_int()
         offs = np.zeros(32, np.int64)
```
